# alshai/pfbwt-f

Hardware: AMD Instinct MI355X
Metric: Gbases/s end-to-end BWT+SA build; bit-exact .bwt/.sa vs reference (higher is better)
Workload: dtype u8 text / u32 indices / u64 hash; 1 GPU; S-32G; L=32000000, H=1000, seed=1000, w=10, p=100, flags=-r, uint_t=64, n=32000010000, r=83625322, input=text resident in HBM, outputs (.bwt, .ssa, .esa) left in HBM, per_rank=single GPU

## Files before the change

pfbwt-f_amd/csrc/common.h:

```cpp
#pragma once
#include <hip/hip_runtime.h>
#include <cstdint>
#include <cstdio>
#include <cstdlib>
#include <cstring>
#include <chrono>
#include <string>
#include <vector>
#include "../../include/pfbwt_hip.h"
#include "devmem.h"
#include "../../include/pfbwt_hip_dev.h"

namespace pfp {

typedef uint32_t idx_t;

constexpr int BLOCK = 256;
constexpr int WAVE = 64;

constexpr uint8_t Dollar = 2, EndOfWord = 1, EndOfDict = 0;

enum KernelId {
    K_TRIGGER_SCAN, K_PHRASE_ENDS, K_PHRASE_HASH, K_PHRASE_HASH_LONG, K_DEDUP_HEADS, K_DEDUP_LONG,
    K_DICT_BUILD, K_RADIX_HIST, K_RADIX_SCATTER, K_SCAN_REDUCE, K_SCAN_SPINE, K_SCAN_APPLY,
    K_SS_INIT_KEYS, K_SS_HEADS, K_SS_MAKE_KEYS, K_SS_WRITE_RANK, K_SS_FLAG_ACTIVE, K_COMPACT,
    K_WORD_RANK, K_PARSE_RANKS, K_DICT_SORTED, K_PBWT_ROWS, K_EMIT_COUNT, K_EMIT, K_RUNS, K_SAMPLES, K_MISC, K_EMIT_BIG, K_FILL, K_CLASS_SORT, K_FASTA, K_EMIT_LARGE, K_REC_PARSE, K_REC_DEDUP, K_REC_ASSEMBLE, K_DOC, K_LCP_PAIRS, K_LCP_LONG, K_LCP_GATHER, K_THR_TILES, K_THR_QUERIES, K_THR_LONG, K_PLCP_BUILD, K_LCP_SPARSE, K_RUN_MASKS, K_MS_INDEX, K_MS_POINTERS, K_MS_BREAKS, K_MS_LONG, K_MS_FILL, K_RI_INDEX, K_RI_SEARCH, K_RI_WALK, K_RI_ROWS,
    K_COUNT_
};
static const char *const kernel_names[K_COUNT_] = {
    "trigger_scan", "phrase_ends", "phrase_hash", "phrase_hash_long", "dedup_heads", "dedup_long",
    "dict_build", "radix_hist", "radix_scatter", "scan_reduce", "scan_spine", "scan_apply",
    "ss_init_keys", "ss_heads", "ss_make_keys", "ss_write_rank", "ss_flag_active", "compact",
    "word_rank", "parse_ranks", "dict_sorted", "pbwt_rows", "emit_count", "emit", "runs", "samples", "misc", "emit_big", "fill", "class_sort", "fasta_strip", "emit_large", "rec_parse", "rec_dedup", "rec_assemble", "doc_array", "lcp_pairs", "lcp_long", "lcp_gather", "thr_tiles", "thr_queries", "thr_long", "plcp_build", "lcp_sparse", "run_masks", "ms_index", "ms_pointers", "ms_breaks", "ms_long", "ms_fill", "ri_index", "ri_search", "ri_walk", "ri_rows"};

struct ProfRec { uint64_t launches = 0; double ms = 0, bytes = 0; };

struct Arena {
    VmRegion vm;
    char *base = nullptr;
    size_t cap = 0, lo = 0, hi = 0, want = 0;
    size_t peak_lo = 0, peak_hi_bytes = 0;
    bool failed = false;
    void reset() { lo = 0; hi = cap; failed = false; }
    void *alloc_lo(size_t bytes)
    {
        size_t a = (lo + 255) & ~(size_t)255;
        if (a + bytes > hi || !vm.commit(a, a + bytes)) { failed = true; want += bytes; return nullptr; }
        lo = a + bytes; if (lo > peak_lo) peak_lo = lo;
        return base + a;
    }
    void *alloc_hi(size_t bytes)
    {
        size_t b = (bytes + 255) & ~(size_t)255;
        if (b > hi || hi - b < lo || !vm.commit(hi - b, hi)) { failed = true; want += bytes; return nullptr; }
        hi -= b; if (cap - hi > peak_hi_bytes) peak_hi_bytes = cap - hi;
        return base + hi;
    }
    void *reserve_lo(size_t bytes)
    {
        size_t a = (lo + 255) & ~(size_t)255;
        if (a + bytes > hi) { failed = true; want += bytes; return nullptr; }
        lo = a + bytes;
        return base + a;
    }
    bool commit_range(const void *p, size_t bytes) { const size_t o = (size_t)((const char *)p - base); return vm.commit(o, o + bytes); }
    size_t offset_of(const void *p) const { return (size_t)((const char *)p - base); }
    size_t mark_hi() const { return hi; }
    void release_hi(size_t m) { hi = m; }
    size_t mark_lo() const { return lo; }
    void release_lo(size_t m) { lo = m; }
};

struct ResultSlot {
    void *p[3] = {nullptr, nullptr, nullptr};
    size_t lo_mark = (size_t)-1, lo_end = 0;
};
struct MsIndex {
    void *thr = nullptr, *lfhead = nullptr; uint8_t *head = nullptr; uint32_t *sorted = nullptr, *sym = nullptr, *dir = nullptr;
    uint32_t B = 0;
};
struct RiIndex {
    MsIndex run; void *pq = nullptr, *pv = nullptr; uint32_t *pdir = nullptr;
    uint32_t PB = 0;
};

struct Tunables {
    int verbose = 0;
    int seg_grid = 768;
    int seg_stage = 1;
    int sort_k = 0;
    int sort_no_table = 0;
    uint32_t class_sort_maxrange = 0;
    int dedup_table_log2 = 0;
    int no_trigger_table = 0;
    uint64_t emit_chunk_rows = 3ULL << 30;
    uint32_t fill_subs = 2;
    int fill_masks = 1;
    int fill_skip = 1;
    uint64_t sample_cap = ~0ULL;
    int no_runaware = 0;
    long big_group_members = -2;
    int force_wide_rows = 0;
    uint64_t ingest_block_bytes = 0;
    int expand_dma = 1;
    int ingest_readers = 0;
    uint32_t emit_group_rows = 4096;
    int dict_text_rounds = -1;
    int force_run_round = 0;
    int int_key_symbols = 3;
    int no_slot_records = 0;
    int group_reduce = 1;
    uint64_t fasta_chunk_bytes = 0;
    int parse_rec = -1;
    int parse_rec_p2 = 4;
    uint64_t parse_rec_min = 1u << 21;
    int parse_rec_depth = 1;
    uint32_t parse_rec_tile_rows = 0;
    int dict_rec = -1;
    int dict_rec_p2 = 16;
    int dedup_variant = -1;
    int64_t dedup_period = 0;
    int64_t dedup_chunk = 0;
    int dedup_packed = 1;
    int scan_waves = 16;
    int dedup_phases = 0;
    int parse_rec_table_log2 = 0;
    uint32_t doc_lds_max = 8192;
    uint32_t lcp_long_min = 512;
    uint32_t thr_long_min = 128;
    uint32_t thr_tile = 1024;
    uint64_t thr_window_rows = 1ULL << 30;
    int ms_dir_log2 = -1;
    uint32_t ms_long_min = 512;
    int ri_dir_log2 = -1;
    int ri_route = 0;
    int plcp_block_log2 = -1;
};

}

struct pfp_ctx {
    int w = 10; uint64_t p = 100; unsigned flags = 0; int device = 0;
    hipStream_t stream = nullptr;
    pfp::Arena arena;
    size_t arena_request = 0;
    uint64_t err_pos = 0; int err_ch = 0;
    pfp::VmRegion text;
    uint8_t *tb = nullptr; size_t tb_cap = 0; uint64_t n = 0; uint64_t text_hint = 0; uint64_t nseq = 0 ;
    struct RowViewPending { const uint8_t *src = nullptr; uint64_t count = 0, len = 0, stride = 0; } view;
    uint64_t left_ctx = 0;
    uint64_t tb_n = 0;
    int stage = 0;
    uint64_t m = 0, dwords = 0, dsize = 0;
    uint64_t *d_ye = nullptr;
    uint32_t *d_pid = nullptr;
    uint32_t *d_parse = nullptr;
    uint8_t *d_last = nullptr;
    uint8_t *d_dict = nullptr;
    uint32_t *d_ws = nullptr;
    uint32_t *d_wordid = nullptr;
    uint32_t *d_wrank = nullptr;
    uint32_t *d_occ = nullptr;
    uint8_t *d_sdict = nullptr;
    uint32_t *d_gsa = nullptr;
    uint8_t *d_sflag = nullptr;
    uint32_t *d_srank = nullptr;
    uint2 *d_grank = nullptr;
    bool gsa_valid = false;
    uint64_t nrows = 0;
    uint8_t *d_bwlast = nullptr; uint32_t *d_ilist = nullptr; uint64_t *d_bwsai = nullptr;
    uint8_t *d_bwl_il = nullptr;
    uint64_t nout = 0, runs = 0, esa_pairs = 0, easy = 0, hard = 0, slice_begin = 0, slice_rows = 0;
    uint8_t *d_bwt = nullptr; void *d_sa = nullptr; void *d_ssa = nullptr; void *d_esa = nullptr;
    bool have_sa = false, have_rssa = false;
    pfp::ResultSlot ma; uint64_t ma_words = 0;
    pfp::ResultSlot da;
    pfp::ResultSlot lcp;
    pfp::ResultSlot thr;
    pfp::ResultSlot msi; pfp::MsIndex msx;
    pfp::ResultSlot ms; uint64_t ms_patterns = 0, ms_bases = 0;
    std::vector<uint64_t> ms_off;
    pfp::ResultSlot rii; pfp::RiIndex rix;
    pfp::ResultSlot ri; uint64_t ri_patterns = 0, ri_reported = 0; int ri_route = 0;
    std::vector<uint64_t> ri_off;
    size_t lo_after_parse = 0, lo_after_pbwt = 0, emit_scratch_mark = 0;
    bool prof_on = false; uint64_t prof_mask = ~0ULL;
    pfp::ProfRec prof[pfp::K_COUNT_];
    struct PendingEv { hipEvent_t a, b; int id; double bytes; };
    std::vector<PendingEv> pending;
    std::vector<hipEvent_t> ev_pool;
    double stage_ms[3] = {0, 0, 0};
    int hip_err = 0;
    uint8_t *hstage[2] = {nullptr, nullptr}; hipEvent_t hstage_ev[2] = {nullptr, nullptr}; bool hstage_used[2] = {false, false};
    pfp::Tunables tun;
    struct FastaIngest {
        uint8_t *raw[2] = {nullptr, nullptr}; size_t rawcap = 0; bool used[2] = {false, false};
        hipStream_t copy = nullptr; bool copy_ready = false; hipEvent_t ev_copied[2] = {nullptr, nullptr}, ev_free[2] = {nullptr, nullptr};
        uint8_t *tiles = nullptr; size_t tiles_cap = 0;
        unsigned long long *d_tot = nullptr, *h_tot = nullptr;
        uint32_t state = 2; bool started = false; uint64_t records = 0;
        std::vector<uint64_t> rec_raw, rec_pos;
    } fa;
    uint8_t *h_bwt = nullptr; void *h_sa = nullptr;
    uint8_t *ing_buf[16] = {};
    uint64_t ing_next_off = 0;
    std::vector<std::string> doc_names; std::vector<uint64_t> doc_starts;
    uint64_t hash_seed = 0x9E3779B97F4A7C15ULL;
    int num_cus = 0;
    uint32_t *d_trigtab = nullptr;
};

namespace pfp {

inline hipEvent_t ev_get(pfp_ctx *c)
{
    if (!c->ev_pool.empty()) { hipEvent_t e = c->ev_pool.back(); c->ev_pool.pop_back(); return e; }
    hipEvent_t e; (void)hipEventCreate(&e); return e;
}
inline void prof_collect(pfp_ctx *c)
{
    if (c->pending.empty()) return;
    (void)hipStreamSynchronize(c->stream);
    for (auto &pe : c->pending) {
        float ms = 0; (void)hipEventElapsedTime(&ms, pe.a, pe.b);
        c->prof[pe.id].launches++; c->prof[pe.id].ms += ms; c->prof[pe.id].bytes += pe.bytes;
        c->ev_pool.push_back(pe.a); c->ev_pool.push_back(pe.b);
    }
    c->pending.clear();
}
struct ProfScope {
    pfp_ctx *c; int id; double bytes; hipEvent_t a = nullptr; bool on = false;
    ProfScope(pfp_ctx *c_, int id_, double bytes_) : c(c_), id(id_), bytes(bytes_)
    {
        on = c->prof_on && ((c->prof_mask >> id) & 1ULL);
        if (on) { a = ev_get(c); (void)hipEventRecord(a, c->stream); }
    }
    ~ProfScope()
    {
        if (on) {
            hipEvent_t b = ev_get(c); (void)hipEventRecord(b, c->stream);
            c->pending.push_back({a, b, id, bytes});
            if (c->pending.size() > 4096) prof_collect(c);
        }
    }
};

#define PFP_LAUNCH(ctx, id, bytes, kernel, grid, ...)                                             \
    do {                                                                                          \
        pfp::ProfScope ps_((ctx), (id), (double)(bytes));                                         \
        if ((ctx)->tun.verbose >= 3) { fprintf(stderr, "[pfbwt_hip] launch %s grid %u\n", #kernel, (unsigned)(grid)); fflush(stderr); } \
        hipLaunchKernelGGL(kernel, dim3((unsigned)(grid)), dim3(pfp::BLOCK), 0, (ctx)->stream, __VA_ARGS__); \
        hipError_t le_ = hipGetLastError();             \
        if ((ctx)->tun.verbose >= 3 && le_ == hipSuccess) le_ = hipStreamSynchronize((ctx)->stream);    \
        if (le_ != hipSuccess) { (ctx)->hip_err = (int)le_; (ctx)->err_ch = (int)le_;                 \
            fprintf(stderr, "[pfbwt_hip] launch of %s failed: %s (%s:%d)\n", #kernel, hipGetErrorString(le_), __FILE__, __LINE__); \
            return PFP_E_HIP; }                                                                       \
    } while (0)

#define PFP_LAUNCH_B(ctx, id, bytes, kernel, grid, block, ...)                                    \
    do {                                                                                          \
        pfp::ProfScope ps_((ctx), (id), (double)(bytes));                                         \
        hipLaunchKernelGGL(kernel, dim3((unsigned)(grid)), dim3((unsigned)(block)), 0, (ctx)->stream, __VA_ARGS__); \
        hipError_t le_ = hipGetLastError();                                                       \
        if (le_ != hipSuccess) { (ctx)->hip_err = (int)le_; (ctx)->err_ch = (int)le_;                 \
            fprintf(stderr, "[pfbwt_hip] launch of %s failed: %s (%s:%d)\n", #kernel, hipGetErrorString(le_), __FILE__, __LINE__); \
            return PFP_E_HIP; }                                                                       \
    } while (0)

#define PFP_HIP(ctx, expr)                                                                        \
    do {                                                                                          \
        hipError_t e_ = (expr);                                                                   \
        if (e_ != hipSuccess) { (ctx)->hip_err = (int)e_; (ctx)->err_ch = (int)e_;                \
            fprintf(stderr, "[pfbwt_hip] %s failed: %s (%s:%d)\n", #expr, hipGetErrorString(e_), __FILE__, __LINE__); \
            return PFP_E_HIP; }                                                                   \
    } while (0)

#define PFP_TRY(expr) do { int rc_ = (expr); if (rc_ != PFP_OK) return rc_; } while (0)

#define PFP_ALLOC_HI(ctx, ptr, T, count)                                                          \
    do { (ptr) = (T *)(ctx)->arena.alloc_hi(sizeof(T) * (size_t)((count) ? (count) : 1));         \
         if (!(ptr)) return PFP_E_NOMEM; } while (0)
#define PFP_ALLOC_LO(ctx, ptr, T, count)                                                          \
    do { (ptr) = (T *)(ctx)->arena.alloc_lo(sizeof(T) * (size_t)((count) ? (count) : 1));         \
         if (!(ptr)) return PFP_E_NOMEM; } while (0)

inline unsigned nblocks(uint64_t items, uint64_t per_block) { return (unsigned)((items + per_block - 1) / per_block); }
inline int bits_for(uint64_t maxval) { int b = 1; while (b < 64 && (maxval >> b)) ++b; return b; }

struct PostResult {
    pfp_ctx *c; ResultSlot &s; size_t mark;
    PostResult(pfp_ctx *c_, ResultSlot &s_) : c(c_), s(s_)
    {
        if (s.lo_mark != (size_t)-1 && c->arena.lo == s.lo_end) c->arena.release_lo(s.lo_mark);
        s = ResultSlot();
        mark = c->arena.mark_lo();
    }
    void commit(void *p0, void *p1 = nullptr, void *p2 = nullptr) { s.p[0] = p0; s.p[1] = p1; s.p[2] = p2; s.lo_mark = mark; s.lo_end = c->arena.mark_lo(); }
};
inline void drop_post_results(pfp_ctx *c) { c->ma = c->da = c->lcp = c->thr = c->msi = c->ms = ResultSlot(); c->ma_words = 0; c->msx = MsIndex(); c->ms_patterns = c->ms_bases = 0; c->ms_off.clear();
    c->rii = c->ri = ResultSlot(); c->rix = RiIndex(); c->ri_patterns = c->ri_reported = 0; c->ri_route = 0; c->ri_off.clear(); }

struct HostTimer {
    std::chrono::steady_clock::time_point t0 = std::chrono::steady_clock::now();
    double ms() const { return std::chrono::duration<double, std::milli>(std::chrono::steady_clock::now() - t0).count(); }
};

}
```

pfbwt-f_amd/csrc/dictrec.h:

```cpp
#pragma once
#include "recsort.h"

namespace pfp {

constexpr int DR_W = 4;
constexpr uint32_t DR_MAX_PHRASE = 1024;

__device__ __forceinline__ uint32_t dr_trigger(const uint8_t *D, uint64_t x, uint32_t p2)
{
    const uint8_t c = D[x];
    if (c == EndOfWord) return 1u;
    if (c == EndOfDict || x < (uint64_t)(DR_W - 1)) return 0u;
    uint32_t v = 0;
#pragma unroll
    for (int k = 0; k < DR_W; ++k) { const uint32_t b = D[x - (DR_W - 1) + k]; if (b <= 1u) return 0u; v = (v << 8) | b; }
    uint32_t h = v * 0x9E3779B1u; h ^= h >> 15; h *= 0x85EBCA77u; h ^= h >> 13;
    return (h % p2 == 0u) ? 1u : 0u;
}
__global__ __launch_bounds__(BLOCK) void k_dr_trig_count(const uint8_t *D, uint64_t N, uint32_t p2, uint32_t *cnt)
{
    __shared__ uint32_t red[4];
    const uint64_t x0 = ((uint64_t)blockIdx.x * BLOCK + threadIdx.x) * 16;
    uint32_t n = 0;
    for (int k = 0; k < 16; ++k) if (x0 + k < N) n += dr_trigger(D, x0 + k, p2);
// ... 46 lines not shown
        if (e == 0ULL) {
            e = atomicCAS(&table[slot], 0ULL, mine);
            if (e == 0ULL) { rep = 1; break; }
        }
        if ((uint32_t)(e >> 32) == tag) {
            const uint32_t r = (uint32_t)e - 1u, ra = ps[r];
            if (pe[r] - ra == b - a) {
                bool eq = true;
                for (uint32_t d = 0; d <= b - a; ++d) if (D[ra + d] != D[a + d]) { eq = false; break; }
                if (eq) break;
            }
        }
        slot = (slot + 1u) & tmask;
    }
    if (probe == REC_MAX_PROBES) atomicExch(overflow, 1u);
    eid[j] = slot; isrep[j] = rep;
}
__global__ __launch_bounds__(BLOCK) void k_dr_rep_keys(const uint8_t *D, const uint32_t *ps, const uint32_t *pe, const uint32_t *replist, uint64_t nw2, uint64_t *keys, uint32_t *vals)
{
    const uint64_t t = (uint64_t)blockIdx.x * BLOCK + threadIdx.x;
    if (t >= nw2) return;
    const uint32_t j = replist[t];
    keys[t] = dr_phrase_hash(D, ps[j], pe[j]); vals[t] = (uint32_t)t;
}
__global__ __launch_bounds__(BLOCK) void k_dr_assign_ids(const uint8_t *D, const uint32_t *sorted_t, const uint32_t *replist, const uint32_t *eid, const uint32_t *ps, const uint32_t *pe, uint64_t nw2,
                                                         uint32_t *slot2id, uint32_t *wrep, uint32_t *wlen1, uint8_t *lastw)
{
    const uint64_t i = (uint64_t)blockIdx.x * BLOCK + threadIdx.x;
    if (i > nw2) return;
    if (i == nw2) { wlen1[i] = 0u; return; }
    const uint32_t j = replist[sorted_t[i]];
    const uint32_t last = D[pe[j]] == EndOfWord ? 1u : 0u;
    slot2id[eid[j]] = (uint32_t)i; wrep[i] = j; lastw[i] = (uint8_t)last;
    wlen1[i] = pe[j] - ps[j] + 1u - last + 1u;
}
__global__ __launch_bounds__(BLOCK) void k_dr_dict_build(const uint8_t *D, const uint32_t *ps, const uint32_t *wrep, const uint32_t *wstart, uint64_t nw2, uint64_t ND, uint8_t *D2, uint32_t *wd2)
{
    const uint64_t i = (uint64_t)blockIdx.x * BLOCK + threadIdx.x;
    if (i > nw2) return;
    if (i == nw2) { D2[ND - 1] = EndOfDict; wd2[ND - 1] = (uint32_t)(nw2 ? nw2 - 1 : 0); return; }
    const uint32_t j = wrep[i], a = ps[j], o = wstart[i], L = wstart[i + 1] - o - 1u;
    for (uint32_t d = 0; d < L; ++d) { D2[o + d] = D[a + d]; wd2[o + d] = (uint32_t)i; }
    D2[o + L] = EndOfWord; wd2[o + L] = (uint32_t)i;
}
__global__ __launch_bounds__(BLOCK) void k_dr_names(const uint8_t *D, const uint32_t *pe, const uint32_t *wordid, const uint32_t *wid2, const uint32_t *wrank2, uint64_t k, uint64_t nwords, uint32_t *P2)
{
    const uint64_t j = (uint64_t)blockIdx.x * BLOCK + threadIdx.x;
    if (j < k) {
        const uint32_t e = pe[j], wj = wordid[e];
        P2[j + wj] = wrank2[wid2[j]] + 2u;
        if (D[e] == EndOfWord) P2[j + wj + 1] = 1u;
    } else if (j == k) P2[k + nwords] = 0u;
}
constexpr uint32_t DR_TIE_CAP = 1024;
__global__ __launch_bounds__(BLOCK) void k_dr_p2_heads(const uint32_t *P2, const uint32_t *SA2, uint64_t n2, uint32_t *headslot, uint8_t *open, uint32_t *nopen)
{
    __shared__ uint32_t red[4];
    const uint64_t s = (uint64_t)blockIdx.x * BLOCK + threadIdx.x;
    uint32_t op = 0u;
    if (s < n2) {
        uint32_t hd = 1u;
        if (s > 0) {
            const uint32_t x = SA2[s], y = SA2[s - 1];
            uint32_t d = 0;
            for (; d < DR_TIE_CAP; ++d) {
                const uint32_t a = x + d < n2 ? P2[x + d] : 0u, b = y + d < n2 ? P2[y + d] : 0u;
                if (a != b) { hd = (a | b) > 1u ? 1u : 0u; break; }
                if (a <= 1u) { hd = 0u; break; }
            }
            if (d == DR_TIE_CAP) { hd = 0u; op = 1u; }
        }
        headslot[s] = hd ? (uint32_t)s : 0u;
        open[s] = (uint8_t)op;
    }
    uint32_t tot;
    (void)block_excl_sum(op, red, &tot);
    if (threadIdx.x == 0 && tot) atomicAdd(nopen, tot);
}
__global__ __launch_bounds__(BLOCK) void k_dr_p2_ends(const uint32_t *P2, uint64_t n2, uint32_t *E)
{
    const uint64_t i = (uint64_t)blockIdx.x * BLOCK + threadIdx.x;
    if (i < n2) E[n2 - 1 - i] = P2[i] <= 1u ? (uint32_t)(n2 - 1 - i) : 0u;
}
__global__ __launch_bounds__(BLOCK) void k_dr_p2_double(const uint32_t *SA2, const uint32_t *rc, const uint32_t *E, uint64_t n2, uint64_t h, uint8_t *open, uint32_t *headslot, uint32_t *nopen)
{
    __shared__ uint32_t red[4];
    const uint64_t s = (uint64_t)blockIdx.x * BLOCK + threadIdx.x;
    uint32_t op = 0u;
    if (s < n2 && open[s]) {
        const uint32_t x = SA2[s], y = SA2[s - 1];
        if (rc[x + h] != rc[y + h]) headslot[s] = (uint32_t)s;
        else if (n2 - 1 - E[n2 - 1 - x] - x >= 2 * h) op = 1u;
        open[s] = (uint8_t)op;
    }
    uint32_t tot;
    (void)block_excl_sum(op, red, &tot);
    if (threadIdx.x == 0 && tot) atomicAdd(nopen, tot);
}
__global__ __launch_bounds__(BLOCK) void k_dr_p2_class(const uint32_t *SA2, const uint32_t *headslot , uint64_t n2, uint32_t *rc)
{
    const uint64_t s = (uint64_t)blockIdx.x * BLOCK + threadIdx.x;
    if (s < n2) rc[SA2[s]] = headslot[s];
}
__global__ __launch_bounds__(BLOCK) void k_dr_list_payload(const uint8_t *D, const uint32_t *inv, const uint32_t *ps, const uint32_t *pe, const uint32_t *wordid, const uint32_t *rc, uint64_t k, uint32_t *ikey, uint32_t *ipos)
{
    const uint64_t e = (uint64_t)blockIdx.x * BLOCK + threadIdx.x;
    if (e >= k) return;
    const uint32_t j = inv[e], en = pe[j];
    ikey[e] = D[en] == EndOfWord ? 0u : rc[j + 1u + wordid[en]];
    const uint32_t x = ps[j];
    ipos[e] = x | ((D[x] > EndOfWord && (x == 0 || D[x - 1] == EndOfWord)) ? 0x80000000u : 0u);
}
__global__ __launch_bounds__(BLOCK) void k_dr_slots(const uint32_t *SA2d, const uint32_t *wd2, const uint32_t *wstart, const uint8_t *lastw, const uint32_t *woff, uint64_t ND, uint32_t *rows, uint32_t *whole, uint32_t *valid)
{
    const uint64_t s = (uint64_t)blockIdx.x * BLOCK + threadIdx.x;
    if (s >= ND) return;
    const uint32_t y = SA2d[s];
    uint32_t v = 0u, r = 0u, wh = 0u;
    if (y + 1 < ND) {
        const uint32_t W = wd2[y], o = y - wstart[W], L = wstart[W + 1] - wstart[W] - 1u;
        v = lastw[W] ? 1u : (o + (uint32_t)DR_W + 1u <= L ? 1u : 0u);
        r = v ? woff[W + 1] - woff[W] : 0u;
        wh = (o == 0u && L > 0u) ? 1u : 0u;
    }
    rows[s] = r; whole[s] = wh; valid[s] = v;
}
__global__ __launch_bounds__(BLOCK) void k_dr_word_ranks(const uint32_t *SA2d, const uint32_t *wd2, const uint32_t *whole, const uint32_t *wpos, uint64_t ND, uint32_t *wrank2)
{
    const uint64_t s = (uint64_t)blockIdx.x * BLOCK + threadIdx.x;
    if (s < ND && whole[s]) wrank2[wd2[SA2d[s]]] = wpos[s];
}
__global__ __launch_bounds__(BLOCK) void k_dr_heads(const uint32_t *vlist, const uint32_t *srank2, uint64_t nv, uint32_t *head)
{
    const uint64_t v = (uint64_t)blockIdx.x * BLOCK + threadIdx.x;
    if (v >= nv) return;
    head[v] = (v == 0 || srank2[vlist[v]] != srank2[vlist[v - 1]]) ? 1u : 0u;
}
__global__ __launch_bounds__(BLOCK) void k_dr_slot_records(const uint32_t *SA2d, const uint32_t *vlist, const uint32_t *rowoff, const uint32_t *head, const uint32_t *hpos, const uint32_t *wd2, const uint32_t *wstart,
                                                           const uint32_t *woff, uint64_t nv, uint4 *srec)
{
    const uint64_t v = (uint64_t)blockIdx.x * BLOCK + threadIdx.x;
    if (v >= nv) return;
    const uint32_t s = vlist[v], y = SA2d[s], W = wd2[y];
    srec[v] = make_uint4(rowoff[s], woff[W], y - wstart[W], hpos[v] + head[v] - 1u);
}
__global__ __launch_bounds__(BLOCK) void k_dr_mark_class_rows(const uint32_t *crow, uint64_t nc, uint32_t *cstart)
{
    const uint64_t ci = (uint64_t)blockIdx.x * BLOCK + threadIdx.x;
    if (ci < nc) cstart[1u + crow[ci]] = 1u;
}
__global__ __launch_bounds__(BLOCK) void k_dr_final_heads(const uint32_t *okey, const uint32_t *cstart, uint64_t N, uint32_t *headslot)
{
    const uint64_t r = (uint64_t)blockIdx.x * BLOCK + threadIdx.x;
    if (r >= N) return;
    const bool hd = r <= 1 || cstart[r] || okey[r] != okey[r - 1];
    headslot[r] = hd ? (uint32_t)r : 0u;
}
inline int dict_sort_pfp(pfp_ctx *c, uint32_t *gsa, uint32_t *srank, uint8_t *sflag, int *taken)
{
    *taken = 0;
    const uint64_t N = c->dsize, nwords = c->dwords;
    const uint8_t *D = c->d_dict;
    const bool forced = c->tun.dict_rec > 0, verbose = c->tun.verbose != 0;
    const uint32_t p2 = c->tun.dict_rec_p2 >= 2 ? (uint32_t)c->tun.dict_rec_p2 : 16u;
    if (N < 64 || N + 64 >= 0x7FFFFFFFULL || !c->d_wordid) return PFP_OK;
    const size_t mk = c->arena.mark_hi();
    HostTimer tm;
    const unsigned gt = nblocks(N, 16 * BLOCK);
    uint32_t *bcnt, *d_cnt;
    PFP_ALLOC_HI(c, bcnt, uint32_t, gt); PFP_ALLOC_HI(c, d_cnt, uint32_t, 16);
    PFP_HIP(c, hipMemsetAsync(d_cnt, 0, 64, c->stream));
    PFP_LAUNCH(c, K_REC_PARSE, N, k_dr_trig_count, gt, D, N, p2, bcnt);
    PFP_TRY((device_scan<uint32_t, 0>(c, bcnt, bcnt, (uint64_t)gt, d_cnt)));
    uint32_t k32 = 0; PFP_TRY(d2h_u32(c, d_cnt, &k32));
    const uint64_t k = k32;
    if (k < nwords || (!forced && k * 6 > N)) { c->arena.release_hi(mk); return PFP_OK; }
    uint32_t *pe, *ps;
    PFP_ALLOC_HI(c, pe, uint32_t, k + 1); PFP_ALLOC_HI(c, ps, uint32_t, k + 1);
    PFP_LAUNCH(c, K_REC_PARSE, N + k * 4, k_dr_trig_write, gt, D, N, p2, (const uint32_t *)bcnt, pe);
    PFP_LAUNCH(c, K_REC_PARSE, k * 9, k_dr_starts, nblocks(k, BLOCK), D, (const uint32_t *)pe, k, ps, d_cnt + 1);
    uint32_t maxlen = 0; PFP_TRY(d2h_u32(c, d_cnt + 1, &maxlen));
    if (maxlen > DR_MAX_PHRASE) {
        if (verbose) fprintf(stderr, "[pfbwt_hip] recursive dictionary sort given up: a level-2 phrase of %u bytes\n", maxlen);
        c->arena.release_hi(mk); return PFP_OK;
    }
    int tl = c->tun.parse_rec_table_log2 > 0 ? c->tun.parse_rec_table_log2 : bits_for(k / 2 + 1023);
    if (tl > 31) tl = 31;
    const uint64_t tsize = 1ULL << tl;
    unsigned long long *table; uint32_t *eid, *isrep, *pos;
    PFP_ALLOC_HI(c, table, unsigned long long, tsize); PFP_ALLOC_HI(c, eid, uint32_t, k); PFP_ALLOC_HI(c, isrep, uint32_t, k); PFP_ALLOC_HI(c, pos, uint32_t, k);
    PFP_HIP(c, hipMemsetAsync(table, 0, tsize * 8, c->stream));
    PFP_LAUNCH(c, K_REC_DEDUP, N * 2 + k * 24, k_dr_dedup, nblocks(k, BLOCK), D, (const uint32_t *)ps, (const uint32_t *)pe, k, table, (uint32_t)(tsize - 1), eid, isrep, d_cnt + 3);
    uint32_t ovf = 0; PFP_TRY(d2h_u32(c, d_cnt + 3, &ovf));
    if (ovf) { if (verbose) fprintf(stderr, "[pfbwt_hip] recursive dictionary sort given up: phrase table too full\n"); c->arena.release_hi(mk); return PFP_OK; }
    uint32_t *replist; PFP_ALLOC_HI(c, replist, uint32_t, k < tsize ? k : tsize);
    PFP_TRY(device_compact(c, nullptr, isrep, k, replist, pos, d_cnt + 4));
    uint32_t nw32 = 0; PFP_TRY(d2h_u32(c, d_cnt + 4, &nw32));
    const uint64_t nw2 = nw32;
    uint32_t *slot2id, *wrep, *wstart, *wid2 = isrep, *inv0, *wid1, *inv1, *woff; uint8_t *lastw;
    PFP_ALLOC_HI(c, slot2id, uint32_t, tsize); PFP_ALLOC_HI(c, wrep, uint32_t, nw2); PFP_ALLOC_HI(c, wstart, uint32_t, nw2 + 1); PFP_ALLOC_HI(c, lastw, uint8_t, nw2 + 1);
    PFP_ALLOC_HI(c, inv0, uint32_t, k); PFP_ALLOC_HI(c, wid1, uint32_t, k); PFP_ALLOC_HI(c, inv1, uint32_t, k); PFP_ALLOC_HI(c, woff, uint32_t, nw2 + 1);
    {
        const size_t mk2 = c->arena.mark_hi();
        uint64_t *hk0, *hk1; uint32_t *hv0, *hv1;
        PFP_ALLOC_HI(c, hk0, uint64_t, nw2); PFP_ALLOC_HI(c, hk1, uint64_t, nw2); PFP_ALLOC_HI(c, hv0, uint32_t, nw2); PFP_ALLOC_HI(c, hv1, uint32_t, nw2);
        PFP_LAUNCH(c, K_REC_DEDUP, nw2 * 40, k_dr_rep_keys, nblocks(nw2, BLOCK), D, (const uint32_t *)ps, (const uint32_t *)pe, (const uint32_t *)replist, nw2, hk0, hv0);
        BitRange hr = {0, 64};
        uint64_t *sk; uint32_t *sv;
        PFP_TRY(radix_sort_pairs<uint64_t>(c, hk0, hv0, hk1, hv1, nw2, &hr, 1, &sk, &sv));
        PFP_LAUNCH(c, K_REC_DEDUP, nw2 * 24, k_dr_assign_ids, nblocks(nw2 + 1, BLOCK), D, (const uint32_t *)sv, (const uint32_t *)replist, (const uint32_t *)eid, (const uint32_t *)ps, (const uint32_t *)pe, nw2, slot2id, wrep, wstart, lastw);
        c->arena.release_hi(mk2);
    }
    PFP_TRY((device_scan<uint32_t, 0>(c, wstart, wstart, nw2 + 1, d_cnt + 5)));
    uint32_t nd32 = 0; PFP_TRY(d2h_u32(c, d_cnt + 5, &nd32));
    const uint64_t ND = (uint64_t)nd32 + 1;
    const uint64_t n2 = k + nwords + 1;
    if (verbose) fprintf(stderr, "[pfbwt_hip] recursive dictionary sort: %llu bytes, %llu words -> %llu level-2 phrases (longest %u), %llu distinct, D2 = %llu bytes (%.1f ms so far)\n",
                         (unsigned long long)N, (unsigned long long)nwords, (unsigned long long)k, maxlen, (unsigned long long)nw2, (unsigned long long)ND, tm.ms());
    if (!forced && (ND * 2 > N)) { c->arena.release_hi(mk); return PFP_OK; }
    PFP_LAUNCH(c, K_REC_DEDUP, k * 16, k_rs_wid, nblocks(k, BLOCK), (const uint32_t *)eid, (const uint32_t *)slot2id, k, wid2, eid, inv0);
    uint32_t *swid, *inv;
    {
        BitRange wr = {0, bits_for(nw2 ? nw2 - 1 : 0)};
        PFP_TRY(radix_sort_pairs<uint32_t>(c, wid2, inv0, wid1, inv1, k, &wr, 1, &swid, &inv));
        PFP_LAUNCH(c, K_REC_PARSE, k * 4, k_rs_list_bounds, nblocks(k, BLOCK), (const uint32_t *)swid, k, nw2, woff);
    }
    const uint32_t *widp = eid;
    uint8_t *D2; uint32_t *wd2, *gsa2, *srank2;
    PFP_ALLOC_HI(c, D2, uint8_t, ND + 64); PFP_ALLOC_HI(c, wd2, uint32_t, ND); PFP_ALLOC_HI(c, gsa2, uint32_t, ND); PFP_ALLOC_HI(c, srank2, uint32_t, ND);
    PFP_HIP(c, hipMemsetAsync(D2 + ND, 0, 64, c->stream));
    PFP_LAUNCH(c, K_REC_PARSE, ND * 6, k_dr_dict_build, nblocks(nw2 + 1, BLOCK), D, (const uint32_t *)ps, (const uint32_t *)wrep, (const uint32_t *)wstart, nw2, ND, D2, wd2);
    {
        const size_t mk2 = c->arena.mark_hi();
        uint64_t *k0, *k1; uint32_t *v0, *v1; uint2 *rj2;
        PFP_ALLOC_HI(c, k0, uint64_t, ND); PFP_ALLOC_HI(c, k1, uint64_t, ND); PFP_ALLOC_HI(c, v0, uint32_t, ND); PFP_ALLOC_HI(c, v1, uint32_t, ND); PFP_ALLOC_HI(c, rj2, uint2, ND);
        PFP_LAUNCH(c, K_SS_INIT_KEYS, ND * 13, k_dict_init_keys, nblocks(ND, DK_TILE), (const uint8_t *)D2, ND, k0, v0);
        BitRange full = {0, DK_KEY_BITS};
        int rounds = 0;
        PFP_TRY(suffix_sort_doubling<true>(c, ND, k0, v0, k1, v1, &full, 1, DK_CHARS, D2, gsa2, (uint32_t *)nullptr, rj2, &rounds, 9, srank2));
        c->arena.release_hi(mk2);
    }
    if (verbose) fprintf(stderr, "[pfbwt_hip]   D2 sorted (%.1f ms so far)\n", tm.ms());
    uint32_t *rows, *whole, *rowoff, *wposs, *wrank2, *P2, *SA2, *R2, *valid, *rc;
    PFP_ALLOC_HI(c, valid, uint32_t, ND); PFP_ALLOC_HI(c, rows, uint32_t, ND); PFP_ALLOC_HI(c, whole, uint32_t, ND); PFP_ALLOC_HI(c, rowoff, uint32_t, ND); PFP_ALLOC_HI(c, wposs, uint32_t, ND);
    PFP_ALLOC_HI(c, wrank2, uint32_t, nw2); PFP_ALLOC_HI(c, P2, uint32_t, n2); PFP_ALLOC_HI(c, SA2, uint32_t, n2); PFP_ALLOC_HI(c, R2, uint32_t, n2); PFP_ALLOC_HI(c, rc, uint32_t, n2);
    PFP_LAUNCH(c, K_REC_PARSE, ND * 28, k_dr_slots, nblocks(ND, BLOCK), (const uint32_t *)gsa2, (const uint32_t *)wd2, (const uint32_t *)wstart, (const uint8_t *)lastw, (const uint32_t *)woff, ND, rows, whole, valid);
    PFP_TRY((device_scan<uint32_t, 0>(c, whole, wposs, ND, nullptr)));
    PFP_LAUNCH(c, K_REC_PARSE, ND * 16, k_dr_word_ranks, nblocks(ND, BLOCK), (const uint32_t *)gsa2, (const uint32_t *)wd2, (const uint32_t *)whole, (const uint32_t *)wposs, ND, wrank2);
    PFP_LAUNCH(c, K_REC_PARSE, k * 16, k_dr_names, nblocks(k + 1, BLOCK), D, (const uint32_t *)pe, (const uint32_t *)c->d_wordid, widp, (const uint32_t *)wrank2, k, nwords, P2);
    {
        int r2 = 0;
        PFP_TRY(sort_int_suffixes(c, P2, n2, nw2 + 1, SA2, R2, &r2, 1, true));
    }
    uint8_t *open; PFP_ALLOC_HI(c, open, uint8_t, n2);
    PFP_HIP(c, hipMemsetAsync(d_cnt + 8, 0, 4, c->stream));
    PFP_LAUNCH(c, K_REC_PARSE, n2 * 17, k_dr_p2_heads, nblocks(n2, BLOCK), (const uint32_t *)P2, (const uint32_t *)SA2, n2, R2 , open, d_cnt + 8);
    PFP_TRY((device_scan<uint32_t, 1>(c, R2, R2, n2, nullptr)));
    PFP_LAUNCH(c, K_REC_PARSE, n2 * 12, k_dr_p2_class, nblocks(n2, BLOCK), (const uint32_t *)SA2, (const uint32_t *)R2, n2, rc);
    uint32_t nopen = 0; PFP_TRY(d2h_u32(c, d_cnt + 8, &nopen));
    if (nopen) {
        const uint32_t open0 = nopen;
        int rounds = 0;
        uint32_t *E; PFP_ALLOC_HI(c, E, uint32_t, n2);
        PFP_LAUNCH(c, K_REC_PARSE, n2 * 8, k_dr_p2_ends, nblocks(n2, BLOCK), (const uint32_t *)P2, n2, E);
        PFP_TRY((device_scan<uint32_t, 1>(c, E, E, n2, nullptr)));
        for (uint64_t h = DR_TIE_CAP; nopen; h *= 2, ++rounds) {
            PFP_HIP(c, hipMemsetAsync(d_cnt + 8, 0, 4, c->stream));
            PFP_LAUNCH(c, K_REC_PARSE, n2 + (uint64_t)nopen * 24, k_dr_p2_double, nblocks(n2, BLOCK), (const uint32_t *)SA2, (const uint32_t *)rc, (const uint32_t *)E, n2, h, open, R2, d_cnt + 8);
            PFP_TRY((device_scan<uint32_t, 1>(c, R2, R2, n2, nullptr)));
            PFP_LAUNCH(c, K_REC_PARSE, n2 * 12, k_dr_p2_class, nblocks(n2, BLOCK), (const uint32_t *)SA2, (const uint32_t *)R2, n2, rc);
            PFP_TRY(d2h_u32(c, d_cnt + 8, &nopen));
        }
        if (verbose) fprintf(stderr, "[pfbwt_hip]   P2 tie classes: %u neighbour pairs agree on %u symbols, resolved in %d doubling rounds\n", open0, DR_TIE_CAP, rounds);
    }
    if (verbose) fprintf(stderr, "[pfbwt_hip]   P2 sorted (%.1f ms so far)\n", tm.ms());
    uint32_t *ikey = SA2, *ipos = P2;
    PFP_LAUNCH(c, K_REC_PARSE, k * 24, k_dr_list_payload, nblocks(k, BLOCK), D, (const uint32_t *)inv, (const uint32_t *)ps, (const uint32_t *)pe, (const uint32_t *)c->d_wordid, (const uint32_t *)rc, k, ikey, ipos);
    PFP_TRY((device_scan<uint32_t, 0>(c, rows, rowoff, ND, d_cnt + 6)));
    uint32_t R32 = 0; PFP_TRY(d2h_u32(c, d_cnt + 6, &R32));
    if ((uint64_t)R32 != N - 1) { c->arena.release_hi(mk); return PFP_E_CORRUPT; }
    uint32_t *vlist, *head, *chead, *crow;
    PFP_ALLOC_HI(c, vlist, uint32_t, ND); PFP_ALLOC_HI(c, head, uint32_t, ND); PFP_ALLOC_HI(c, chead, uint32_t, ND + 1); PFP_ALLOC_HI(c, crow, uint32_t, ND + 1);
    PFP_TRY(device_compact(c, nullptr, valid, ND, vlist, wposs, d_cnt + 7));
    uint32_t nv32 = 0; PFP_TRY(d2h_u32(c, d_cnt + 7, &nv32));
    const uint64_t nv = nv32;
    uint4 *srec; PFP_ALLOC_HI(c, srec, uint4, nv);
    PFP_LAUNCH(c, K_REC_PARSE, nv * 12, k_dr_heads, nblocks(nv, BLOCK), (const uint32_t *)vlist, (const uint32_t *)srank2, nv, head);
    PFP_HIP(c, hipMemsetAsync(d_cnt, 0, 32, c->stream));
    PFP_TRY(device_compact(c, nullptr, head, nv, chead, wposs, d_cnt));
    PFP_LAUNCH(c, K_REC_PARSE, nv * 44, k_dr_slot_records, nblocks(nv, BLOCK), (const uint32_t *)gsa2, (const uint32_t *)vlist, (const uint32_t *)rowoff, (const uint32_t *)head, (const uint32_t *)wposs, (const uint32_t *)wd2,
               (const uint32_t *)wstart, (const uint32_t *)woff, nv, srec);
    uint32_t nc32 = 0; PFP_TRY(d2h_u32(c, d_cnt, &nc32));
    const uint64_t nc = nc32;
    PFP_LAUNCH(c, K_REC_PARSE, nc * 24, k_rs_class_rows, nblocks(nc + 1, BLOCK), (const uint32_t *)chead, (const uint4 *)srec, nc, nv, N - 1, crow, chead + nc);
    uint32_t tile_rows = c->tun.parse_rec_tile_rows ? c->tun.parse_rec_tile_rows : (uint32_t)RS_TILE;
    if (tile_rows > (uint32_t)RS_TILE) tile_rows = RS_TILE;
    if (tile_rows < 2) tile_rows = 2;
    const int keybits = bits_for(n2);
    uint32_t *bigc, *okey, *cstart;
    PFP_ALLOC_HI(c, bigc, uint32_t, nc + 1); PFP_ALLOC_HI(c, okey, uint32_t, N); PFP_ALLOC_HI(c, cstart, uint32_t, N + 1);
    PFP_HIP(c, hipMemsetAsync(cstart, 0, (N + 1) * 4, c->stream));
    const unsigned ga = nblocks(N - 1, RS_TILE / 2);
    PFP_LAUNCH(c, K_REC_ASSEMBLE, (N - 1) * 16 + nv * 16, (k_rs_assemble<false, true>), ga, (const uint4 *)srec, (const uint32_t *)chead, (const uint32_t *)crow, (uint32_t)nc, (const uint32_t *)ikey, (const uint32_t *)ipos,
               keybits, tile_rows, gsa, (uint32_t *)nullptr, bigc, d_cnt + 1, okey, sflag);
    PFP_LAUNCH(c, K_MISC, 8, k_rs_first_row, 1, gsa, (uint32_t *)nullptr, N);
    uint32_t nb32 = 0; PFP_TRY(d2h_u32(c, d_cnt + 1, &nb32));
    if (nb32) {
        const uint64_t nb = nb32;
        uint32_t *bigoff; PFP_ALLOC_HI(c, bigoff, uint32_t, nb + 1);
        PFP_LAUNCH(c, K_REC_PARSE, nb * 12, k_rs_big_sizes, nblocks(nb + 1, BLOCK), (const uint32_t *)bigc, nb, (const uint32_t *)crow, bigoff);
        PFP_TRY((device_scan<uint32_t, 0>(c, bigoff, bigoff, nb + 1, d_cnt + 2)));
        uint32_t nbr32 = 0; PFP_TRY(d2h_u32(c, d_cnt + 2, &nbr32));
        const uint64_t nbr = nbr32;
        if (verbose) fprintf(stderr, "[pfbwt_hip]   assembly: %llu classes with more than %u rows (%llu rows) through the global sort\n", (unsigned long long)nb, tile_rows, (unsigned long long)nbr);
        uint64_t *bk0, *bk1; uint32_t *bv0, *bv1;
        PFP_ALLOC_HI(c, bk0, uint64_t, nbr); PFP_ALLOC_HI(c, bk1, uint64_t, nbr); PFP_ALLOC_HI(c, bv0, uint32_t, nbr); PFP_ALLOC_HI(c, bv1, uint32_t, nbr);
        PFP_LAUNCH(c, K_REC_PARSE, nbr * 40, k_rs_big_rows, nblocks(nbr, BLOCK), (const uint32_t *)bigc, (const uint32_t *)bigoff, (uint32_t)nb, nbr, (const uint32_t *)crow, (const uint32_t *)chead, (const uint4 *)srec,
                   (const uint32_t *)ikey, (const uint32_t *)ipos, bk0, bv0, 1);
        BitRange br[2] = {{0, keybits}, {32, 32 + bits_for(nb - 1)}};
        uint64_t *sk; uint32_t *sv;
        PFP_TRY(radix_sort_pairs<uint64_t>(c, bk0, bv0, bk1, bv1, nbr, br, 2, &sk, &sv));
        PFP_LAUNCH(c, K_REC_PARSE, nbr * 24, (k_rs_big_store<false, true>), nblocks(nbr, BLOCK), (const uint64_t *)sk, (const uint32_t *)sv, nbr, (const uint32_t *)bigc, (const uint32_t *)bigoff, (const uint32_t *)crow, gsa,
                   (uint32_t *)nullptr, okey, sflag);
    }
    PFP_LAUNCH(c, K_REC_PARSE, nc * 8, k_dr_mark_class_rows, nblocks(nc, BLOCK), (const uint32_t *)crow, nc, cstart);
    PFP_LAUNCH(c, K_REC_PARSE, N * 12, k_dr_final_heads, nblocks(N, BLOCK), (const uint32_t *)okey, (const uint32_t *)cstart, N, srank);
    PFP_TRY((device_scan<uint32_t, 1>(c, srank, srank, N, nullptr)));
    PFP_HIP(c, hipMemsetAsync(sflag, 0, 1, c->stream));
    PFP_HIP(c, hipStreamSynchronize(c->stream));
    if (verbose) fprintf(stderr, "[pfbwt_hip]   dictionary assembled: %llu slots, %llu D2 classes (%.1f ms)\n", (unsigned long long)nv, (unsigned long long)nc, tm.ms());
    c->arena.release_hi(mk);
    *taken = 1;
    return PFP_OK;
}

}
```

pfbwt-f_amd/csrc/pfbwt_hip.hip:

```cpp
#include "common.h"
#include "prims.h"
#include "parse.h"
#include "fasta.h"
#include "sufsort.h"
#include "recsort.h"
#include "dictrec.h"
#include "emit.h"
#include "markers.h"
#include "docarray.h"
#include "lcparray.h"
#include "thresholds.h"
#include "matchstats.h"
#include "runindex.h"
#include <algorithm>
#include <functional>
#include <map>
#include <sched.h>
#include <thread>
#if defined(__SSE2__)
#include <emmintrin.h>
#endif

using namespace pfp;

#ifndef PFP_BACKEND_NAME
#define PFP_BACKEND_NAME "hip-gfx950"
#endif

static int ensure_arena(pfp_ctx *c, uint64_t n_hint)
{
    size_t want = c->arena_request ? c->arena_request : (size_t)(96ULL * n_hint + (64ULL << 20));
    if (!c->arena_request) {
        size_t fr = 0, tot = 0;
        if (hipMemGetInfo(&fr, &tot) == hipSuccess) {
            const size_t avail = fr + c->arena.vm.committed;
            const size_t cap = avail - avail / 16;
            if (want > cap) want = cap;
        }
    }
    want &= ~(size_t)4095;
    if (c->arena.base && c->arena.cap >= want) return PFP_OK;
    VmRegion nv;
    if (nv.reserve(want, c->device) != hipSuccess) { c->arena.want = want; return PFP_E_NOMEM; }
    if (c->arena.base) { PFP_HIP(c, hipStreamSynchronize(c->stream)); (void)hipDeviceSynchronize(); c->arena.vm.destroy(); c->arena.base = nullptr; c->arena.cap = 0; }
    c->arena.vm = nv; nv.base = nullptr;
    c->arena.base = c->arena.vm.base; c->arena.cap = want; c->arena.reset();
    return PFP_OK;
}

static int ensure_text(pfp_ctx *c, uint64_t need_n)
{
    const size_t need = 16 + (((size_t)need_n + 4095) / 4096) * 4096 + 4096 + 64;
    if (c->tb && c->tb_cap >= need) return PFP_OK;
    if (!c->text.live() || need > c->text.va_bytes) {
        size_t fr = 0, tot = 0;
        if (hipMemGetInfo(&fr, &tot) != hipSuccess) { (void)hipGetLastError(); tot = (size_t)1 << 38; }
        size_t va = c->text_hint ? (size_t)c->text_hint + (size_t)c->text_hint / 8 + ((size_t)64 << 20) : (4 * need > ((size_t)64 << 20) ? 4 * need : ((size_t)64 << 20));
        if (!c->text_hint && c->text.live() && va < 2 * c->text.va_bytes) va = 2 * c->text.va_bytes;
        if (!c->text_hint && va > tot && tot > need + need / 4) va = tot;
        if (va < need) va = need + need / 4;
        VmRegion nr;
        if (nr.reserve(va, c->device) != hipSuccess) return PFP_E_NOMEM;
        if (c->tb) {
            if (!nr.commit(0, 16 + (size_t)c->n)) { nr.destroy(); return PFP_E_NOMEM; }
            PFP_HIP(c, hipMemcpyAsync(nr.base, c->tb, 16 + (size_t)c->n, hipMemcpyDeviceToDevice, c->stream));
            PFP_HIP(c, hipStreamSynchronize(c->stream));
            c->text.destroy();
        }
        c->text = nr; nr.base = nullptr;
        c->tb = (uint8_t *)c->text.base; c->tb_cap = 0;
    }
    if (!c->text.commit(0, need)) return PFP_E_NOMEM;
    c->tb_cap = c->text.vmm ? (c->text.lo_edge < c->text.va_bytes ? c->text.lo_edge : c->text.va_bytes) : c->text.va_bytes;
    return PFP_OK;
}

static void reset_results(pfp_ctx *c)
{
    c->stage = 0; c->n = 0; c->nseq = 0; c->tb_n = 0; c->left_ctx = 0; c->view.src = nullptr; c->m = c->dwords = c->dsize = 0; c->nrows = 0; c->nout = c->runs = c->esa_pairs = 0;
    c->gsa_valid = false; c->d_wrank = nullptr; c->d_bwt = nullptr; c->d_sa = c->d_ssa = c->d_esa = nullptr;
    c->d_bwlast = nullptr; c->d_ilist = nullptr; c->d_bwsai = nullptr; c->d_bwl_il = nullptr;
    drop_post_results(c);
    c->d_ye = nullptr; c->d_pid = nullptr; c->d_parse = nullptr; c->d_last = nullptr; c->d_dict = nullptr; c->d_ws = nullptr; c->d_wordid = nullptr;
    c->d_occ = nullptr; c->d_sdict = nullptr; c->d_gsa = nullptr; c->d_grank = nullptr; c->d_srank = nullptr; c->d_sflag = nullptr;
    c->arena.reset();
    c->fa.started = false; c->fa.state = 2; c->fa.records = 0; c->fa.rec_raw.clear(); c->fa.rec_pos.clear();
}

static const char *const tunable_names[] = {"verbose", "seg_grid", "seg_stage", "sort_k", "sort_no_table", "class_sort_maxrange", "dedup_table_log2", "no_trigger_table",
                                            "emit_chunk_rows", "fill_subs", "sample_cap", "no_runaware", "big_group_members", "force_wide_rows", "fasta_chunk_bytes", "ingest_block_bytes", "emit_group_rows", "no_slot_records", "dict_text_rounds", "int_key_symbols", "force_run_round",
                                            "ingest_readers", "expand_dma", "parse_rec", "parse_rec_p2", "parse_rec_min", "parse_rec_depth", "parse_rec_tile_rows", "parse_rec_table_log2", "dict_rec", "dict_rec_p2", "dedup_variant", "dedup_phases", "dedup_period", "dedup_chunk", "doc_lds_max", "dedup_packed", "group_reduce", "scan_waves", "lcp_long_min", "thr_long_min", "thr_tile", "thr_window_rows", "plcp_block_log2", "fill_masks", "fill_skip", "ms_dir_log2", "ms_long_min", "ri_dir_log2", "ri_route"};
static int set_tunable(pfp_ctx *c, const char *key, long long v)
{
    Tunables &t = c->tun;
    if (!strcmp(key, "verbose")) t.verbose = (int)v;
    else if (!strcmp(key, "seg_grid")) t.seg_grid = (int)v;
    else if (!strcmp(key, "seg_stage")) t.seg_stage = (int)v;
    else if (!strcmp(key, "sort_k")) t.sort_k = (int)v;
    else if (!strcmp(key, "sort_no_table")) t.sort_no_table = (int)v;
    else if (!strcmp(key, "class_sort_maxrange")) t.class_sort_maxrange = (uint32_t)v;
    else if (!strcmp(key, "dedup_table_log2")) t.dedup_table_log2 = (int)v;
    else if (!strcmp(key, "no_trigger_table")) t.no_trigger_table = (int)v;
    else if (!strcmp(key, "emit_chunk_rows")) t.emit_chunk_rows = v > 0 ? (uint64_t)v : (3ULL << 30);
    else if (!strcmp(key, "fill_subs")) t.fill_subs = (uint32_t)v;
    else if (!strcmp(key, "fill_masks")) t.fill_masks = (int)v;
    else if (!strcmp(key, "fill_skip")) t.fill_skip = (int)v;
    else if (!strcmp(key, "sample_cap")) t.sample_cap = v < 0 ? ~0ULL : (uint64_t)v;
    else if (!strcmp(key, "no_runaware")) t.no_runaware = (int)v;
    else if (!strcmp(key, "big_group_members")) t.big_group_members = (long)v;
    else if (!strcmp(key, "force_wide_rows")) t.force_wide_rows = (int)v;
    else if (!strcmp(key, "fasta_chunk_bytes")) t.fasta_chunk_bytes = v > 0 ? (uint64_t)v : 0;
    else if (!strcmp(key, "ingest_block_bytes")) t.ingest_block_bytes = v > 0 ? (uint64_t)v : 0;
    else if (!strcmp(key, "emit_group_rows")) t.emit_group_rows = v > 0 ? (uint32_t)v : 0u;
    else if (!strcmp(key, "no_slot_records")) t.no_slot_records = (int)v;
    else if (!strcmp(key, "dict_text_rounds")) t.dict_text_rounds = (int)v;
    else if (!strcmp(key, "int_key_symbols")) t.int_key_symbols = (int)v;
    else if (!strcmp(key, "force_run_round")) t.force_run_round = (int)v;
    else if (!strcmp(key, "ingest_readers")) t.ingest_readers = (int)v;
    else if (!strcmp(key, "expand_dma")) t.expand_dma = (int)v;
    else if (!strcmp(key, "parse_rec")) t.parse_rec = (int)v;
    else if (!strcmp(key, "parse_rec_p2")) t.parse_rec_p2 = (int)v;
    else if (!strcmp(key, "parse_rec_min")) t.parse_rec_min = v > 0 ? (uint64_t)v : 0;
    else if (!strcmp(key, "parse_rec_depth")) t.parse_rec_depth = (int)v;
    else if (!strcmp(key, "parse_rec_tile_rows")) t.parse_rec_tile_rows = v > 0 ? (uint32_t)v : 0u;
    else if (!strcmp(key, "parse_rec_table_log2")) t.parse_rec_table_log2 = (int)v;
    else if (!strcmp(key, "dict_rec")) t.dict_rec = (int)v;
    else if (!strcmp(key, "dict_rec_p2")) t.dict_rec_p2 = (int)v;
    else if (!strcmp(key, "dedup_variant")) t.dedup_variant = (int)v;
    else if (!strcmp(key, "dedup_phases")) t.dedup_phases = (int)v;
    else if (!strcmp(key, "dedup_packed")) t.dedup_packed = (int)v;
    else if (!strcmp(key, "group_reduce")) t.group_reduce = (int)v;
    else if (!strcmp(key, "scan_waves")) t.scan_waves = (int)v;
    else if (!strcmp(key, "dedup_period")) t.dedup_period = (int64_t)v;
    else if (!strcmp(key, "dedup_chunk")) t.dedup_chunk = (int64_t)v;
    else if (!strcmp(key, "doc_lds_max")) t.doc_lds_max = v < 2 ? 2u : v > (long long)DOC_LDS_CAP ? DOC_LDS_CAP : (uint32_t)v;
    else if (!strcmp(key, "lcp_long_min")) t.lcp_long_min = v < 16 ? 16u : v > (1LL << 30) ? (1u << 30) : (((uint32_t)v + 15u) & ~15u);
    else if (!strcmp(key, "thr_long_min")) t.thr_long_min = v < 1 ? 1u : v > (1LL << 30) ? (1u << 30) : (uint32_t)v;
    else if (!strcmp(key, "thr_tile")) { uint32_t p2 = 16; while (p2 < (1u << 20) && (long long)p2 < v) p2 *= 2; t.thr_tile = p2; }
    else if (!strcmp(key, "thr_window_rows")) t.thr_window_rows = v < 1 ? (1ULL << 30) : (uint64_t)v;
    else if (!strcmp(key, "plcp_block_log2")) t.plcp_block_log2 = v < 0 ? -1 : v > PLCP_BLOCK_LOG2_MAX ? PLCP_BLOCK_LOG2_MAX : (int)v;
    else if (!strcmp(key, "ms_dir_log2")) t.ms_dir_log2 = v < 0 ? -1 : v > MS_DIR_LOG2_MAX ? MS_DIR_LOG2_MAX : (int)v;
    else if (!strcmp(key, "ms_long_min")) t.ms_long_min = v < 1 ? 1u : v > (1LL << 30) ? (1u << 30) : (uint32_t)v;
    else if (!strcmp(key, "ri_dir_log2")) t.ri_dir_log2 = v < 0 ? -1 : v > RI_DIR_LOG2_MAX ? RI_DIR_LOG2_MAX : (int)v;
    else if (!strcmp(key, "ri_route")) t.ri_route = v < 0 ? 0 : v > 2 ? 2 : (int)v;
    else return PFP_E_ARG;
    return PFP_OK;
}
static void load_tunables_from_env(pfp_ctx *c)
{
    if (getenv("PFP_VERBOSE")) c->tun.verbose = 1;
    const char *hooks = getenv("PFP_TEST_HOOKS");
    if (!hooks || strcmp(hooks, "1")) return;
    for (const char *name : tunable_names) {
        char env[64] = "PFP_"; size_t k = 4;
        for (const char *q = name; *q && k + 1 < sizeof env; ++q) env[k++] = (char)((*q >= 'a' && *q <= 'z') ? *q - 32 : *q);
        env[k] = 0;
        const char *e = getenv(env);
        if (e) (void)set_tunable(c, name, *e ? atoll(e) : 1LL);
    }
}

extern "C" {

const char *pfp_backend(void) { return PFP_BACKEND_NAME; }
int pfp_debug_set(pfp_ctx *c, const char *key, long long value) { return (c && key) ? set_tunable(c, key, value) : PFP_E_ARG; }

const char *pfp_strerror(int s)
{
    switch (s) {
    case PFP_OK: return "ok";
    case PFP_E_ARG: return "invalid argument";
    case PFP_E_INVALID_CHAR: return "error, invalid character";
    case PFP_E_TOO_LARGE: return "input too long for 32-bit device indices";
    case PFP_E_NOMEM: return "device workspace exhausted";
    case PFP_E_HIP: return "HIP runtime error";
    case PFP_E_ONE_WORD: return "error: only one dict word total. Re-run with a smaller p modulus";
    case PFP_E_STATE: return "call order violated";
    case PFP_E_CORRUPT: return "something went wrong!";
    case PFP_E_IO: return "failed to open file!";
    default: return "unknown status";
    }
}

pfp_ctx *pfp_create(int w, uint64_t p, unsigned flags, int device, uint64_t workspace_bytes, int *status)
{
    int st = PFP_OK;
    pfp_ctx *c = nullptr;
    if (w < 1 || w > 32 || p == 0) st = PFP_E_ARG;
    else {
        int ndev = 0;
        if (hipGetDeviceCount(&ndev) != hipSuccess || ndev <= 0 || device < 0 || device >= ndev) st = PFP_E_HIP;
        else if (hipSetDevice(device) != hipSuccess) st = PFP_E_HIP;
        else {
            c = new pfp_ctx();
            c->w = w; c->p = p; c->flags = flags; c->device = device; c->arena_request = (size_t)workspace_bytes;
            load_tunables_from_env(c);
            if (hipStreamCreateWithFlags(&c->stream, hipStreamNonBlocking) != hipSuccess) { delete c; c = nullptr; st = PFP_E_HIP; }
        }
    }
    if (status) *status = st;
    return c;
}

void pfp_destroy(pfp_ctx *c)
{
    if (!c) return;
    (void)hipSetDevice(c->device);
    if (c->stream) (void)hipStreamSynchronize(c->stream);
    (void)hipDeviceSynchronize();
    prof_collect(c);
    for (auto e : c->ev_pool) (void)hipEventDestroy(e);
    c->text.destroy();
    for (int k = 0; k < 2; ++k) { if (c->fa.raw[k]) (void)hipFree(c->fa.raw[k]); if (c->fa.ev_copied[k]) (void)hipEventDestroy(c->fa.ev_copied[k]); if (c->fa.ev_free[k]) (void)hipEventDestroy(c->fa.ev_free[k]); }
    if (c->fa.tiles) (void)hipFree(c->fa.tiles);
    if (c->fa.d_tot) (void)hipFree(c->fa.d_tot);
    if (c->fa.h_tot) (void)hipHostFree(c->fa.h_tot);
    if (c->fa.copy_ready) (void)hipStreamDestroy(c->fa.copy);
    for (auto &q : c->ing_buf) if (q) (void)hipHostFree(q);
    if (c->d_trigtab) (void)hipFree(c->d_trigtab);
    for (int k = 0; k < 2; ++k) { if (c->hstage[k]) (void)hipHostFree(c->hstage[k]); if (c->hstage_ev[k]) (void)hipEventDestroy(c->hstage_ev[k]); }
    c->arena.vm.destroy();
    if (c->stream) (void)hipStreamDestroy(c->stream);
    delete c;
}

int pfp_error_detail(pfp_ctx *c, uint64_t *pos, int *ch)
{
    if (!c) return PFP_E_ARG;
    if (pos) *pos = c->err_pos;
    if (ch) *ch = c->err_ch;
    return PFP_OK;
}
uint64_t pfp_workspace_needed(pfp_ctx *c) { return c ? (uint64_t)(c->arena.cap + c->arena.want) : 0; }
int pfp_reset(pfp_ctx *c)
{
    if (!c) return PFP_E_ARG;
    PFP_HIP(c, hipSetDevice(c->device));
    PFP_HIP(c, hipStreamSynchronize(c->stream));
    reset_results(c);
    return PFP_OK;
}

int pfp_profile_enable(pfp_ctx *c, int on) { if (!c) return PFP_E_ARG; prof_collect(c); c->prof_on = on != 0; c->prof_mask = ~0ULL; return PFP_OK; }
int pfp_profile_select(pfp_ctx *c, const char *kernel)
{
    if (!c || !kernel) return PFP_E_ARG;
    prof_collect(c);
    for (int i = 0; i < K_COUNT_; ++i) if (!strcmp(kernel, kernel_names[i])) { c->prof_on = true; c->prof_mask = 1ULL << i; return PFP_OK; }
    return PFP_E_ARG;
}
int pfp_profile_reset(pfp_ctx *c) { if (!c) return PFP_E_ARG; prof_collect(c); for (auto &r : c->prof) r = ProfRec(); return PFP_OK; }
int pfp_profile_get(pfp_ctx *c, int idx, const char **name, uint64_t *launches, double *ms, double *bytes)
{
    if (!c || idx < 0 || idx >= K_COUNT_) return PFP_E_ARG;
    prof_collect(c);
    if (name) *name = kernel_names[idx];
    if (launches) *launches = c->prof[idx].launches;
    if (ms) *ms = c->prof[idx].ms;
    if (bytes) *bytes = c->prof[idx].bytes;
    return PFP_OK;
}
int pfp_stage_ms(pfp_ctx *c, double out[3]) { if (!c || !out) return PFP_E_ARG; for (int i = 0; i < 3; ++i) out[i] = c->stage_ms[i]; return PFP_OK; }

constexpr size_t STAGE_BYTES = (size_t)32 << 20;
static bool host_pointer_is_pinned(const void *p)
{
    hipPointerAttribute_t a;
    if (hipPointerGetAttributes(&a, p) == hipSuccess) return a.type == hipMemoryTypeHost;
    (void)hipGetLastError();
    return false;
}
static int h2d_copy(pfp_ctx *c, uint8_t *dst, const uint8_t *src, uint64_t len, bool *in_flight = nullptr)
{
    if (in_flight) *in_flight = false;
    if (!len) return PFP_OK;
    if (host_pointer_is_pinned(src)) { PFP_HIP(c, hipMemcpyAsync(dst, src, (size_t)len, hipMemcpyHostToDevice, c->stream)); if (in_flight) *in_flight = true; else PFP_HIP(c, hipStreamSynchronize(c->stream)); return PFP_OK; }
    if (len <= ((size_t)1 << 16)) { PFP_HIP(c, hipMemcpyAsync(dst, src, (size_t)len, hipMemcpyHostToDevice, c->stream)); PFP_HIP(c, hipStreamSynchronize(c->stream)); return PFP_OK; }
    for (int k = 0; k < 2; ++k) if (!c->hstage[k]) {
        PFP_HIP(c, hipHostMalloc((void **)&c->hstage[k], STAGE_BYTES, hipHostMallocDefault));
        PFP_HIP(c, hipEventCreate(&c->hstage_ev[k]));
    }
    int k = 0;
    for (uint64_t off = 0; off < len; off += STAGE_BYTES, k ^= 1) {
        const size_t chunk = (size_t)(len - off < STAGE_BYTES ? len - off : STAGE_BYTES);
        if (c->hstage_used[k]) PFP_HIP(c, hipEventSynchronize(c->hstage_ev[k]));
        memcpy(c->hstage[k], src + off, chunk);
        PFP_HIP(c, hipMemcpyAsync(dst + off, c->hstage[k], chunk, hipMemcpyHostToDevice, c->stream));
        PFP_HIP(c, hipEventRecord(c->hstage_ev[k], c->stream));
        c->hstage_used[k] = true;
    }
    return PFP_OK;
}
static int feed_common(pfp_ctx *c, const void *src, uint64_t len, int end_of_seq, hipMemcpyKind kind)
{
    if (!c || (!src && len)) return PFP_E_ARG;
    PFP_HIP(c, hipSetDevice(c->device));
    if (c->stage != 0) reset_results(c);
    const uint64_t add = len + (end_of_seq ? (uint64_t)c->w : 0);
    if (c->n + add + (uint64_t)c->w + 64 >= ((c->flags & PFP_FLAG_U64) ? (1ULL << 40) : 0xFFFFFFFFULL)) return PFP_E_TOO_LARGE;
    PFP_TRY(ensure_text(c, c->n + add + (uint64_t)c->w));
    bool in_flight = false;
    if (len && kind == hipMemcpyHostToDevice) PFP_TRY(h2d_copy(c, c->tb + 16 + c->n, (const uint8_t *)src, len, &in_flight));
    else if (len) PFP_HIP(c, hipMemcpyAsync(c->tb + 16 + c->n, src, (size_t)len, kind, c->stream));
    c->n += len;
    if (end_of_seq) {
        ++c->nseq;
        PFP_HIP(c, hipMemsetAsync(c->tb + 16 + c->n, 'A', (size_t)c->w, c->stream));
        c->n += (uint64_t)c->w;
    }
    if (in_flight || (len && kind == hipMemcpyDeviceToDevice)) PFP_HIP(c, hipStreamSynchronize(c->stream));
    c->tb_n = c->n;
    return PFP_OK;
}
int pfp_parse_reopen(pfp_ctx *c)
{
    if (!c) return PFP_E_ARG;
    PFP_HIP(c, hipSetDevice(c->device));
    if (c->stage == 0) return PFP_OK;
    if (!c->tb || !c->tb_n || c->tb_n != c->n) return PFP_E_STATE;
    PFP_HIP(c, hipStreamSynchronize(c->stream));
    const uint64_t n = c->n, nseq = c->nseq;
    reset_results(c);
    c->nseq = nseq;
    c->n = c->tb_n = n;
    return PFP_OK;
}
static int flush_view(pfp_ctx *c);
int pfp_text_view(pfp_ctx *c, const uint8_t **d_text, uint64_t *n)
{
    if (!c || !d_text || !n) return PFP_E_ARG;
    PFP_TRY(flush_view(c));
    if (!c->tb || c->tb_n != c->n) { *d_text = nullptr; *n = 0; return PFP_OK; }
    PFP_HIP(c, hipSetDevice(c->device));
    PFP_HIP(c, hipStreamSynchronize(c->stream));
    *d_text = c->tb + 16; *n = c->n;
    return PFP_OK;
}
int pfp_parse_feed_left_context(pfp_ctx *c)
{
    if (!c) return PFP_E_ARG;
    if (c->stage != 0) { PFP_HIP(c, hipSetDevice(c->device)); reset_results(c); }
    if (c->n != 0) return PFP_E_STATE;
    const std::vector<uint8_t> a((size_t)c->w, (uint8_t)'A');
    PFP_TRY(feed_common(c, a.data(), a.size(), 0, hipMemcpyHostToDevice));
    c->left_ctx = (uint64_t)c->w;
    return PFP_OK;
}
static int flush_view(pfp_ctx *c)
{
    if (!c->view.src) return PFP_OK;
    const uint64_t count = c->view.count, len = c->view.len;
    const uint64_t blocks_per_row = ((len + 15) / 16 + BLOCK - 1) / BLOCK;
    PFP_LAUNCH(c, K_MISC, 2 * count * len, k_feed_batch, count * blocks_per_row, c->view.src, count, len, c->view.stride, c->w, c->tb + 16);
    c->view.src = nullptr;
    return PFP_OK;
}
int pfp_parse_feed_device_view(pfp_ctx *c, const void *d_bases, uint64_t count, uint64_t len, uint64_t stride)
{
    if (!c || !d_bases || !count || !len || stride < len) return PFP_E_ARG;
    PFP_HIP(c, hipSetDevice(c->device));
    if (c->stage != 0) reset_results(c);
    if (c->n != 0) return PFP_E_STATE;
    const uint64_t pitch = len + (uint64_t)c->w, add = count * pitch;
    if (add + (uint64_t)c->w + 64 >= ((c->flags & PFP_FLAG_U64) ? (1ULL << 40) : 0xFFFFFFFFULL)) return PFP_E_TOO_LARGE;
    const uint64_t blocks_per_row = ((len + 15) / 16 + BLOCK - 1) / BLOCK;
    if (count * blocks_per_row >= 0x7FFFFFFFULL) return PFP_E_TOO_LARGE;
    PFP_TRY(ensure_text(c, add + (uint64_t)c->w));
    c->view.src = (const uint8_t *)d_bases; c->view.count = count; c->view.len = len; c->view.stride = stride;
    c->n = add; c->tb_n = c->n; c->nseq = count;
    return PFP_OK;
}
int pfp_parse_feed(pfp_ctx *c, const uint8_t *bases, uint64_t len, int end_of_seq) { if (c) PFP_TRY(flush_view(c)); return feed_common(c, bases, len, end_of_seq, hipMemcpyHostToDevice); }
int pfp_parse_feed_device(pfp_ctx *c, const void *d_bases, uint64_t len, int end_of_seq) { if (c) PFP_TRY(flush_view(c)); return feed_common(c, d_bases, len, end_of_seq, hipMemcpyDeviceToDevice); }
int pfp_parse_feed_device_batch(pfp_ctx *c, const void *d_bases, uint64_t count, uint64_t len, uint64_t stride)
{
    if (!c || (!d_bases && count && len) || stride < len) return PFP_E_ARG;
    if (!count) return PFP_OK;
    PFP_TRY(flush_view(c));
    if (!len) { for (uint64_t k = 0; k < count; ++k) PFP_TRY(feed_common(c, nullptr, 0, 1, hipMemcpyDeviceToDevice)); return PFP_OK; }
    PFP_HIP(c, hipSetDevice(c->device));
    if (c->stage != 0) reset_results(c);
    const uint64_t pitch = len + (uint64_t)c->w, add = count * pitch;
    if (c->n + add + (uint64_t)c->w + 64 >= ((c->flags & PFP_FLAG_U64) ? (1ULL << 40) : 0xFFFFFFFFULL)) return PFP_E_TOO_LARGE;
    PFP_TRY(ensure_text(c, c->n + add + (uint64_t)c->w));
    uint8_t *dst = c->tb + 16 + c->n;
    const uint64_t blocks_per_row = ((len + 15) / 16 + BLOCK - 1) / BLOCK;
    if (count * blocks_per_row >= 0x7FFFFFFFULL) return PFP_E_TOO_LARGE;
    PFP_LAUNCH(c, K_MISC, 2 * count * len, k_feed_batch, count * blocks_per_row, (const uint8_t *)d_bases, count, len, stride, c->w, dst);
    c->n += add; c->tb_n = c->n; c->nseq += count;
    return PFP_OK;
}

int pfp_parse_feed_batch(pfp_ctx *c, const uint8_t *bases, uint64_t count, uint64_t len, uint64_t stride)
{
    if (!c || (!bases && count && len) || stride < len) return PFP_E_ARG;
    if (!count) return PFP_OK;
    PFP_TRY(flush_view(c));
    if (!len || !host_pointer_is_pinned(bases)) {
        for (uint64_t k = 0; k < count; ++k) PFP_TRY(feed_common(c, bases + k * stride, len, 1, hipMemcpyHostToDevice));
        return PFP_OK;
    }
    PFP_HIP(c, hipSetDevice(c->device));
    if (c->stage != 0) reset_results(c);
    const uint64_t pitch = len + (uint64_t)c->w, add = count * pitch;
    if (c->n + add + (uint64_t)c->w + 64 >= ((c->flags & PFP_FLAG_U64) ? (1ULL << 40) : 0xFFFFFFFFULL)) return PFP_E_TOO_LARGE;
    PFP_TRY(ensure_text(c, c->n + add + (uint64_t)c->w));
    uint8_t *dst = c->tb + 16 + c->n;
    for (uint64_t k = 0; k < count; ++k) PFP_HIP(c, hipMemcpyAsync(dst + k * pitch, bases + k * stride, (size_t)len, hipMemcpyHostToDevice, c->stream));
    PFP_LAUNCH(c, K_MISC, count * (uint64_t)c->w, k_pad_rows, nblocks(count * (uint64_t)c->w, BLOCK), dst, count, len, pitch, c->w);
    PFP_HIP(c, hipStreamSynchronize(c->stream));
    c->n += add; c->tb_n = c->n; c->nseq += count;
    return PFP_OK;
}

constexpr size_t FA_RAW_MAX = (size_t)256 << 20, FA_RAW_MIN = (size_t)1 << 20;
int pfp_parse_reserve(pfp_ctx *c, uint64_t text_bytes)
{
    if (!c) return PFP_E_ARG;
    if (!c->text.live()) c->text_hint = text_bytes;
    return PFP_OK;
}
static int ensure_copy_stream(pfp_ctx *c)
{
    auto &f = c->fa;
    if (f.copy_ready) return PFP_OK;
    PFP_HIP(c, hipStreamCreateWithFlags(&f.copy, hipStreamNonBlocking));
    f.copy_ready = true;
// ... 1442 lines not shown
```

pfbwt-f_amd/csrc/recsort.h:

```cpp
#pragma once
#include "sufsort.h"

namespace pfp {

constexpr uint32_t REC_MAX_PHRASE = 1024;
constexpr int RS_TRIG_PER = 16;
constexpr int RS_TRIG_TILE = BLOCK * RS_TRIG_PER;

__device__ __forceinline__ uint32_t rs_trigger(uint32_t s, uint32_t p2)
{
    uint32_t h = s * 0x9E3779B1u; h ^= h >> 15; h *= 0x85EBCA77u; h ^= h >> 13;
    return (h % p2 == 0u) ? 1u : 0u;
}
__device__ __forceinline__ uint32_t rs_trig_mask16(const uint32_t *S, uint64_t N, uint64_t i0, uint32_t p2)
{
    uint32_t m = 0;
    if (i0 + RS_TRIG_PER <= N) {
        const uint4 *q = reinterpret_cast<const uint4 *>(S + i0);
#pragma unroll
        for (int v = 0; v < 4; ++v) {
            const uint4 a = q[v];
            m |= (rs_trigger(a.x, p2) | (rs_trigger(a.y, p2) << 1) | (rs_trigger(a.z, p2) << 2) | (rs_trigger(a.w, p2) << 3)) << (4 * v);
        }
    } else {
        for (int k = 0; k < RS_TRIG_PER; ++k) if (i0 + k < N) m |= rs_trigger(S[i0 + k], p2) << k;
    }
    if (i0 == 0) m &= ~1u;
    if (N - 1 >= i0 && N - 1 < i0 + RS_TRIG_PER) m |= 1u << (uint32_t)(N - 1 - i0);
    return m;
}
__global__ __launch_bounds__(BLOCK) void k_rs_trig_count(const uint32_t *S, uint64_t N, uint32_t p2, uint32_t *cnt)
{
    __shared__ uint32_t red[4];
    const uint64_t i0 = ((uint64_t)blockIdx.x * BLOCK + threadIdx.x) * RS_TRIG_PER;
    const uint32_t m = i0 < N ? rs_trig_mask16(S, N, i0, p2) : 0u;
    uint32_t tot;
    (void)block_excl_sum((uint32_t)__popc(m), red, &tot);
    if (threadIdx.x == 0) cnt[blockIdx.x] = tot;
}
__global__ __launch_bounds__(BLOCK) void k_rs_trig_write(const uint32_t *S, uint64_t N, uint32_t p2, const uint32_t *blockoff, uint32_t *ps)
{
    __shared__ uint32_t red[4];
    const uint64_t i0 = ((uint64_t)blockIdx.x * BLOCK + threadIdx.x) * RS_TRIG_PER;
    uint32_t m = i0 < N ? rs_trig_mask16(S, N, i0, p2) : 0u;
    uint32_t tot;
    uint32_t o = 1u + blockoff[blockIdx.x] + block_excl_sum((uint32_t)__popc(m), red, &tot);
    while (m) { const int b = __ffs((int)m) - 1; ps[o++] = (uint32_t)(i0 + (uint32_t)b); m &= m - 1u; }
    if (blockIdx.x == 0 && threadIdx.x == 0) ps[0] = 0u;
}
__global__ __launch_bounds__(BLOCK) void k_rs_max_phrase(const uint32_t *ps, uint64_t k, uint32_t *out)
{
    __shared__ uint32_t red[4];
    const uint64_t j = (uint64_t)blockIdx.x * BLOCK + threadIdx.x;
    const uint32_t len = j < k ? ps[j + 1] - ps[j] + 1u : 0u;
    uint32_t tot;
    (void)block_incl_max(len, red, &tot);
    if (threadIdx.x == 0 && tot > *(volatile uint32_t *)out) atomicMax(out, tot);
}

constexpr uint32_t REC_MAX_PROBES = 128;
__device__ __forceinline__ uint64_t rs_phrase_hash(const uint32_t *S, uint32_t a, uint32_t b)
{
    uint64_t h = 0x243F6A8885A308D3ULL;
    for (uint32_t i = a; i <= b; ++i) { h = (h ^ S[i]) * 0x9E3779B97F4A7C15ULL; h ^= h >> 29; }
    h *= 0xBF58476D1CE4E5B9ULL; h ^= h >> 32;
    return h;
}
__global__ __launch_bounds__(BLOCK) void k_rs_dedup(const uint32_t *S, const uint32_t *ps, uint64_t k, unsigned long long *table, uint32_t tmask, uint32_t *eid, uint32_t *isrep, uint32_t *overflow)
{
    const uint64_t j = (uint64_t)blockIdx.x * BLOCK + threadIdx.x;
    if (j >= k) return;
    const uint32_t a = ps[j], b = ps[j + 1];
    const uint64_t h = rs_phrase_hash(S, a, b);
    const uint32_t tag = (uint32_t)(h >> 32);
    const unsigned long long mine = ((unsigned long long)tag << 32) | (unsigned long long)(a + 1u);
    uint32_t slot = (uint32_t)h & tmask, rep = 0, probe = 0;
    for (; probe < REC_MAX_PROBES; ++probe) {
        unsigned long long e = table[slot];
        if (e == 0ULL) {
            e = atomicCAS(&table[slot], 0ULL, mine);
            if (e == 0ULL) { rep = 1; break; }
        }
        if ((uint32_t)(e >> 32) == tag) {
            const uint32_t ra = (uint32_t)e - 1u;
            bool eq = true;
            for (uint32_t d = 0; d <= b - a; ++d) if (S[ra + d] != S[a + d]) { eq = false; break; }
            if (eq) break;
        }
        slot = (slot + 1u) & tmask;
    }
    if (probe == REC_MAX_PROBES) atomicExch(overflow, 1u);
    eid[j] = slot; isrep[j] = rep;
}
__global__ __launch_bounds__(BLOCK) void k_rs_rep_keys(const uint32_t *S, const uint32_t *ps, const uint32_t *replist, uint64_t nw, uint64_t k, uint64_t *keys, uint32_t *vals)
{
    const uint64_t t = (uint64_t)blockIdx.x * BLOCK + threadIdx.x;
    if (t >= nw) return;
    const uint32_t j = replist[t];
    keys[t] = (uint64_t)j + 1 == k ? ~0ULL : (rs_phrase_hash(S, ps[j], ps[j + 1]) >> 1);
    vals[t] = (uint32_t)t;
}
__global__ __launch_bounds__(BLOCK) void k_rs_assign_ids(const uint32_t *sorted_t, const uint32_t *replist, const uint32_t *eid, const uint32_t *ps, uint64_t nw, uint32_t *slot2id, uint32_t *wrep, uint32_t *wlen1)
{
    const uint64_t i = (uint64_t)blockIdx.x * BLOCK + threadIdx.x;
    if (i > nw) return;
    if (i == nw) { wlen1[i] = 0u; return; }
    const uint32_t j = replist[sorted_t[i]];
    slot2id[eid[j]] = (uint32_t)i; wrep[i] = j;
    wlen1[i] = ps[j + 1] - ps[j] + 2u;
}
__global__ __launch_bounds__(BLOCK) void k_rs_wid(const uint32_t *eid, const uint32_t *slot2id, uint64_t k, uint32_t *wid, uint32_t *wid_keep, uint32_t *idx)
{
    const uint64_t j = (uint64_t)blockIdx.x * BLOCK + threadIdx.x;
    if (j < k) { const uint32_t id = slot2id[eid[j]]; wid[j] = id; wid_keep[j] = id; idx[j] = (uint32_t)j; }
}
__global__ __launch_bounds__(BLOCK) void k_rs_dict_build(const uint32_t *S, const uint32_t *ps, const uint32_t *wrep, const uint32_t *wstart, uint64_t nw, uint32_t *D, uint32_t *wd)
{
    const uint64_t i = (uint64_t)blockIdx.x * BLOCK + threadIdx.x;
    if (i >= nw) return;
    const uint32_t j = wrep[i], a = ps[j], L = ps[j + 1] - a + 1u, o = wstart[i];
    for (uint32_t d = 0; d < L; ++d) { D[o + d] = S[a + d] + 2u; wd[o + d] = (uint32_t)i; }
    D[o + L] = i + 1 == nw ? 0u : 1u; wd[o + L] = (uint32_t)i;
}
__global__ __launch_bounds__(BLOCK) void k_rs_list_bounds(const uint32_t *skeys, uint64_t k, uint64_t nw, uint32_t *woff)
{
    const uint64_t e = (uint64_t)blockIdx.x * BLOCK + threadIdx.x;
    if (e >= k) return;
    const uint32_t id = skeys[e];
    if (e == 0 || skeys[e - 1] != id) woff[id] = (uint32_t)e;
    if (e + 1 == k) woff[nw] = (uint32_t)k;
}
__global__ __launch_bounds__(BLOCK) void k_rs_slots(const uint32_t *SAD, const uint32_t *wd, const uint32_t *wstart, const uint32_t *woff, uint64_t ND, uint32_t *rows, uint32_t *whole, uint32_t *valid)
{
    const uint64_t s = (uint64_t)blockIdx.x * BLOCK + threadIdx.x;
    if (s >= ND) return;
    const uint32_t x = SAD[s], i = wd[x], o = x - wstart[i], L = wstart[i + 1] - wstart[i] - 1u;
    rows[s] = o + 1u < L ? woff[i + 1] - woff[i] : 0u;
    valid[s] = o + 1u < L ? 1u : 0u;
    whole[s] = o == 0u ? 1u : 0u;
}
__global__ __launch_bounds__(BLOCK) void k_rs_word_ranks(const uint32_t *SAD, const uint32_t *wd, const uint32_t *whole, const uint32_t *wpos, uint64_t ND, uint32_t *wrank)
{
    const uint64_t s = (uint64_t)blockIdx.x * BLOCK + threadIdx.x;
    if (s < ND && whole[s]) wrank[wd[SAD[s]]] = wpos[s] + 1u;
}
__global__ __launch_bounds__(BLOCK) void k_rs_names(const uint32_t *wid, const uint32_t *wrank, uint64_t k, uint32_t *P2)
{
    const uint64_t j = (uint64_t)blockIdx.x * BLOCK + threadIdx.x;
    if (j < k) P2[j] = wrank[wid[j]];
    else if (j == k) P2[j] = 0u;
}
__global__ __launch_bounds__(BLOCK) void k_rs_list_payload(const uint32_t *inv, const uint32_t *R2, const uint32_t *ps, uint64_t k, uint32_t *ikey, uint32_t *ipos)
{
    const uint64_t e = (uint64_t)blockIdx.x * BLOCK + threadIdx.x;
    if (e >= k) return;
    const uint32_t j = inv[e];
    ikey[e] = R2[j + 1]; ipos[e] = ps[j];
}
__global__ __launch_bounds__(BLOCK) void k_rs_heads(const uint32_t *D, const uint32_t *SAD, const uint32_t *vlist, uint64_t nv, uint32_t *head)
{
    const uint64_t v = (uint64_t)blockIdx.x * BLOCK + threadIdx.x;
    if (v >= nv) return;
    const uint32_t s = vlist[v];
    const uint32_t sp = v ? vlist[v - 1] : 0u;
    uint32_t hd = (v == 0 || sp + 1u != s) ? 1u : 0u;
    uint32_t x = SAD[s], y = SAD[s ? s - 1 : 0];
    if (!hd) {
        for (uint32_t d = 0; d <= REC_MAX_PHRASE + 1u; ++d) {
            const uint32_t a = D[x + d], b = D[y + d];
            if (a != b) { hd = (a | b) > 1u ? 1u : 0u; break; }
            if (a <= 1u) break;
        }
    }
    head[v] = hd;
}
__global__ __launch_bounds__(BLOCK) void k_rs_slot_records(const uint32_t *SAD, const uint32_t *vlist, const uint32_t *rowoff, const uint32_t *head, const uint32_t *hpos , const uint32_t *wd, const uint32_t *wstart,
                                                            const uint32_t *woff, uint64_t nv, uint4 *srec)
{
    const uint64_t v = (uint64_t)blockIdx.x * BLOCK + threadIdx.x;
    if (v >= nv) return;
    const uint32_t s = vlist[v], x = SAD[s], i = wd[x];
    srec[v] = make_uint4(rowoff[s], woff[i], x - wstart[i], hpos[v] + head[v] - 1u);
}
__global__ __launch_bounds__(BLOCK) void k_rs_class_rows(const uint32_t *chead, const uint4 *srec, uint64_t nc, uint64_t nv, uint64_t R, uint32_t *crow, uint32_t *chead_end)
{
    const uint64_t ci = (uint64_t)blockIdx.x * BLOCK + threadIdx.x;
    if (ci < nc) crow[ci] = srec[chead[ci]].x;
    else if (ci == nc) { crow[ci] = (uint32_t)R; *chead_end = (uint32_t)nv; }
}

__device__ __forceinline__ uint32_t rs_lower_bound(const uint32_t *a, uint32_t lo, uint32_t hi, uint64_t key)
{
    while (lo < hi) { const uint32_t mid = lo + ((hi - lo) >> 1); if ((uint64_t)a[mid] < key) lo = mid + 1; else hi = mid; }
    return lo;
}

template <int NB> __device__ __forceinline__ void rs_same_digit_lanes(uint32_t d, uint32_t &plo, uint32_t &phi)
{
#pragma unroll
    for (int bb = 0; bb < NB; ++bb) {
        const uint32_t neg = (uint32_t)(((int32_t)(d << (31 - bb))) >> 31);
        const unsigned long long m = __builtin_amdgcn_ballot_w64(neg != 0u);
        plo &= ~((uint32_t)m ^ neg); phi &= ~((uint32_t)(m >> 32) ^ neg);
    }
}

constexpr int RA_DB = 9, RA_RADIX = 1 << RA_DB;
template <bool RANK, bool KEYOUT> __global__ __launch_bounds__(BLOCK) void k_rs_assemble(const uint4 *srec, const uint32_t *chead , const uint32_t *crow , uint32_t nc,
                                                                            const uint32_t *ikey, const uint32_t *ipos, int keybits, uint32_t tile_rows, uint32_t *SA, uint32_t *rank,
                                                                            uint32_t *bigc, uint32_t *nbig, uint32_t *okey ,
                                                                            uint8_t *oflag )
{
    constexpr int ITEMS = RS_ITEMS, TILE = RS_TILE;
    constexpr uint32_t STEP = TILE / 2;
    __shared__ uint32_t wh[BLOCK / WAVE][RA_RADIX];
    __shared__ uint64_t skeys[TILE];
    __shared__ uint16_t sidx[TILE];
    __shared__ uint16_t srow[TILE + 1];
    __shared__ uint32_t red[4];
    __shared__ uint32_t ctl[4];
    const int lane = threadIdx.x & 63, wave = threadIdx.x >> 6;
    const uint64_t w0 = (uint64_t)blockIdx.x * STEP;
    if (threadIdx.x == 0) { ctl[0] = rs_lower_bound(crow, 0u, nc, w0); ctl[1] = rs_lower_bound(crow, 0u, nc, w0 + STEP); }
    __syncthreads();
    uint32_t ci = ctl[0];
    const uint32_t ci1 = ctl[1];
    while (ci < ci1) {
        __syncthreads();
        if (threadIdx.x == 0) {
            const uint64_t lim = (uint64_t)crow[ci] + tile_rows;
            uint32_t lo = ci, hi = ci1;
            while (lo < hi) { const uint32_t mid = lo + ((hi - lo + 1) >> 1); if ((uint64_t)crow[mid] <= lim) lo = mid; else hi = mid - 1; }
            ctl[2] = lo;
            if (lo == ci) bigc[atomicAdd(nbig, 1u)] = ci;
        }
        __syncthreads();
        const uint32_t cj = ctl[2];
        if (cj == ci) { ++ci; continue; }
        const uint32_t r0 = crow[ci], n = crow[cj] - r0, v0 = chead[ci], ns = chead[cj] - v0;
        for (uint32_t t = threadIdx.x; t < ns; t += BLOCK) srow[t] = (uint16_t)(srec[v0 + t].x - r0);
        if (threadIdx.x == 0) srow[ns] = (uint16_t)n;
        __syncthreads();
        const uint32_t nit = (n + BLOCK - 1) / BLOCK;
        uint32_t xi[ITEMS];
#pragma unroll
        for (int it = 0; it < ITEMS; ++it) {
            const uint32_t i = threadIdx.x + (uint32_t)it * BLOCK;
            xi[it] = 0u;
            if (i < n) {
                uint32_t lo = 0, hi = ns - 1;
                while (lo < hi) { const uint32_t mid = lo + ((hi - lo + 1) >> 1); if (srow[mid] <= i) lo = mid; else hi = mid - 1; }
                const uint4 rec = srec[v0 + lo];
                const uint32_t e = rec.y + (i - (rec.x - r0));
                xi[it] = KEYOUT ? (rec.z ? (ipos[e] & 0x7FFFFFFFu) + rec.z : ipos[e]) : ipos[e] + rec.z;
                skeys[i] = ((uint64_t)(rec.w - ci) << keybits) | ikey[e];
                sidx[i] = (uint16_t)i;
            }
        }
        for (uint32_t i = n + threadIdx.x; i < nit * BLOCK; i += BLOCK) { skeys[i] = ~0ULL; sidx[i] = (uint16_t)i; }
        __syncthreads();
        int tbits = keybits;
        for (uint32_t hs = cj - 1 - ci; hs; hs >>= 1) ++tbits;
        const int npass = (tbits + RA_DB - 1) / RA_DB;
        const uint32_t base = (uint32_t)wave * (nit * WAVE) + lane;
        for (int p = 0; p < npass; ++p) {
            const int sh = RA_DB * p;
            uint64_t kk[ITEMS]; uint16_t vv[ITEMS]; unsigned dg[ITEMS];
#pragma unroll
            for (int w = 0; w < BLOCK / WAVE; ++w) { wh[w][threadIdx.x] = 0; wh[w][threadIdx.x + BLOCK] = 0; }
            __syncthreads();
#pragma unroll
            for (int it = 0; it < ITEMS; ++it) {
                if ((uint32_t)it < nit) {
                    const uint32_t i = base + (uint32_t)it * WAVE;
                    kk[it] = skeys[i]; vv[it] = sidx[i];
                    const uint32_t d = (uint32_t)(kk[it] >> sh) & (RA_RADIX - 1);
                    uint32_t plo = 0xFFFFFFFFu, phi = 0xFFFFFFFFu;
                    rs_same_digit_lanes<RA_DB>(d, plo, phi);
                    const int leader = plo ? __builtin_ctz(plo) : 32 + __builtin_ctz(phi);
                    uint32_t old = 0;
                    if (lane == leader) { old = wh[wave][d]; wh[wave][d] = old + (uint32_t)__builtin_popcount(plo) + (uint32_t)__builtin_popcount(phi); }
                    old = __shfl(old, leader);
                    dg[it] = d | ((old + __builtin_amdgcn_mbcnt_hi(phi, __builtin_amdgcn_mbcnt_lo(plo, 0u))) << RA_DB);
                }
            }
            __syncthreads();
            {
                const unsigned d0 = 2u * threadIdx.x;
                uint32_t c0[BLOCK / WAVE], c1[BLOCK / WAVE]; uint32_t total = 0;
#pragma unroll
                for (int w = 0; w < BLOCK / WAVE; ++w) { const uint2 q = *reinterpret_cast<const uint2 *>(&wh[w][d0]); c0[w] = q.x; c1[w] = q.y; total += q.x + q.y; }
                uint32_t tt;
                uint32_t run = block_excl_sum(total, red, &tt);
                uint32_t o0[BLOCK / WAVE];
#pragma unroll
                for (int w = 0; w < BLOCK / WAVE; ++w) { o0[w] = run; run += c0[w]; }
#pragma unroll
                for (int w = 0; w < BLOCK / WAVE; ++w) { *reinterpret_cast<uint2 *>(&wh[w][d0]) = make_uint2(o0[w], run); run += c1[w]; }
            }
            __syncthreads();
#pragma unroll
            for (int it = 0; it < ITEMS; ++it) {
                if ((uint32_t)it < nit) {
                    const uint32_t li = wh[wave][dg[it] & (RA_RADIX - 1)] + (dg[it] >> RA_DB);
                    skeys[li] = kk[it]; sidx[li] = vv[it];
                }
            }
            __syncthreads();
        }
        if (KEYOUT) {
            const uint64_t km = keybits >= 32 ? 0xFFFFFFFFULL : ((1ULL << keybits) - 1ULL);
            for (uint32_t i = threadIdx.x; i < n; i += BLOCK) okey[1u + r0 + i] = (uint32_t)(skeys[i] & km);
            __syncthreads();
        }
        uint32_t *sx = reinterpret_cast<uint32_t *>(skeys);
#pragma unroll
        for (int it = 0; it < ITEMS; ++it) { const uint32_t i = threadIdx.x + (uint32_t)it * BLOCK; if (i < n) sx[i] = xi[it]; }
        __syncthreads();
        for (uint32_t i = threadIdx.x; i < n; i += BLOCK) {
            uint32_t x = sx[sidx[i]];
            if (KEYOUT) { oflag[1u + r0 + i] = (uint8_t)(x >> 31); x &= 0x7FFFFFFFu; }
            SA[1u + r0 + i] = x;
            if (RANK) rank[x] = 1u + r0 + i;
        }
        ci = cj;
    }
}

__global__ __launch_bounds__(BLOCK) void k_rs_big_sizes(const uint32_t *bigc, uint64_t nb, const uint32_t *crow, uint32_t *sizes)
{
    const uint64_t b = (uint64_t)blockIdx.x * BLOCK + threadIdx.x;
    if (b < nb) sizes[b] = crow[bigc[b] + 1] - crow[bigc[b]];
    else if (b == nb) sizes[b] = 0u;
}
__global__ __launch_bounds__(BLOCK) void k_rs_big_rows(const uint32_t *bigc, const uint32_t *bigoff , uint32_t nb, uint64_t nbr, const uint32_t *crow, const uint32_t *chead, const uint4 *srec,
                                                       const uint32_t *ikey, const uint32_t *ipos, uint64_t *keys, uint32_t *vals, int flagged )
{
    const uint64_t q = (uint64_t)blockIdx.x * BLOCK + threadIdx.x;
    if (q >= nbr) return;
    uint32_t lo = 0, hi = nb - 1;
    while (lo < hi) { const uint32_t mid = lo + ((hi - lo + 1) >> 1); if ((uint64_t)bigoff[mid] <= q) lo = mid; else hi = mid - 1; }
    const uint32_t b = lo, c = bigc[b], row = crow[c] + (uint32_t)(q - bigoff[b]);
    uint32_t vl = chead[c], vh = chead[c + 1] - 1;
    while (vl < vh) { const uint32_t mid = vl + ((vh - vl + 1) >> 1); if (srec[mid].x <= row) vl = mid; else vh = mid - 1; }
    const uint4 rec = srec[vl];
    const uint32_t e = rec.y + (row - rec.x);
    keys[q] = ((uint64_t)b << 32) | ikey[e];
    vals[q] = flagged ? (rec.z ? (ipos[e] & 0x7FFFFFFFu) + rec.z : ipos[e]) : ipos[e] + rec.z;
}
template <bool RANK, bool KEYOUT> __global__ __launch_bounds__(BLOCK) void k_rs_big_store(const uint64_t *keys, const uint32_t *vals, uint64_t nbr, const uint32_t *bigc, const uint32_t *bigoff, const uint32_t *crow, uint32_t *SA, uint32_t *rank, uint32_t *okey, uint8_t *oflag)
{
    const uint64_t q = (uint64_t)blockIdx.x * BLOCK + threadIdx.x;
    if (q >= nbr) return;
    const uint32_t b = (uint32_t)(keys[q] >> 32);
    const uint32_t row = crow[bigc[b]] + (uint32_t)(q - bigoff[b]);
    uint32_t x = vals[q];
    if (KEYOUT) { oflag[1u + row] = (uint8_t)(x >> 31); x &= 0x7FFFFFFFu; }
    SA[1u + row] = x;
    if (RANK) rank[x] = 1u + row;
    if (KEYOUT) okey[1u + row] = (uint32_t)keys[q];
}
__global__ __launch_bounds__(BLOCK) void k_rs_first_row(uint32_t *SA, uint32_t *rank, uint64_t N)
{
    if (blockIdx.x == 0 && threadIdx.x == 0) { SA[0] = (uint32_t)(N - 1); if (rank) rank[N - 1] = 0u; }
}

inline int sort_int_suffixes(pfp_ctx *c, const uint32_t *dS, uint64_t N, uint64_t maxsym, uint32_t *SA, uint32_t *rank, int *rounds, int depth = 0, bool want_rank = true);

inline int sort_int_suffixes_doubling(pfp_ctx *c, const uint32_t *dS, uint64_t N, uint64_t maxsym, uint32_t *SA, uint32_t *rank, int *rounds)
{
    const size_t mk = c->arena.mark_hi();
    uint64_t *k0, *k1; uint32_t *v0, *v1;
    PFP_ALLOC_HI(c, k0, uint64_t, N); PFP_ALLOC_HI(c, k1, uint64_t, N);
    PFP_ALLOC_HI(c, v0, uint32_t, N); PFP_ALLOC_HI(c, v1, uint32_t, N);
    const int sb = bits_for(maxsym);
    const int nsym = (c->tun.int_key_symbols == 3 && 3 * sb <= 64) ? 3 : 2;
    PFP_LAUNCH(c, K_SS_INIT_KEYS, N * 16, k_int_init_keys, nblocks(N, BLOCK), dS, N, sb, nsym, k0, v0);
    BitRange rr = {0, nsym * sb};
    PFP_TRY(suffix_sort_doubling<false>(c, N, k0, v0, k1, v1, &rr, 1, (uint32_t)nsym, (const uint8_t *)nullptr, SA, rank, (uint2 *)nullptr, rounds));
    c->arena.release_hi(mk);
    return PFP_OK;
}

inline int suffix_sort_pfp(pfp_ctx *c, const uint32_t *dS, uint64_t N, uint64_t maxsym, uint32_t *SA, uint32_t *rank , int depth, int *taken)
{
    *taken = 0;
    const bool forced = c->tun.parse_rec > 0, verbose = c->tun.verbose != 0;
    const uint32_t p2 = c->tun.parse_rec_p2 >= 2 ? (uint32_t)c->tun.parse_rec_p2 : 4u;
    if (N < 8 || N + 64 >= 0xFFFFFFFFULL || maxsym + 2 >= 0xFFFFFFFFULL) return PFP_OK;
    const size_t mk = c->arena.mark_hi();
    HostTimer tm;
    const unsigned gt = nblocks(N, RS_TRIG_TILE);
    uint32_t *bcnt, *d_cnt;
    PFP_ALLOC_HI(c, bcnt, uint32_t, gt); PFP_ALLOC_HI(c, d_cnt, uint32_t, 8);
    PFP_HIP(c, hipMemsetAsync(d_cnt, 0, 32, c->stream));
    PFP_LAUNCH(c, K_REC_PARSE, N * 4, k_rs_trig_count, gt, dS, N, p2, bcnt);
    PFP_TRY((device_scan<uint32_t, 0>(c, bcnt, bcnt, (uint64_t)gt, d_cnt)));
    uint32_t k32 = 0; PFP_TRY(d2h_u32(c, d_cnt, &k32));
    const uint64_t k = k32;
    if (k < 2 || (!forced && k * 2 > N)) { c->arena.release_hi(mk); return PFP_OK; }
    if (N + 2 * k >= 0xFFFFFFFFULL) {
        if (verbose) fprintf(stderr, "[pfbwt_hip] recursive parse sort given up: N + 2 * %llu phrases do not fit 32 bits\n", (unsigned long long)k);
        c->arena.release_hi(mk); return PFP_OK;
    }
    uint32_t *ps; PFP_ALLOC_HI(c, ps, uint32_t, k + 1);
    PFP_LAUNCH(c, K_REC_PARSE, N * 4 + k * 4, k_rs_trig_write, gt, dS, N, p2, (const uint32_t *)bcnt, ps);
    PFP_LAUNCH(c, K_REC_PARSE, k * 4, k_rs_max_phrase, nblocks(k, BLOCK), (const uint32_t *)ps, k, d_cnt + 1);
    uint32_t maxlen = 0; PFP_TRY(d2h_u32(c, d_cnt + 1, &maxlen));
    if (maxlen > REC_MAX_PHRASE) {
        if (verbose) fprintf(stderr, "[pfbwt_hip] recursive parse sort given up: a level-2 phrase of %u symbols\n", maxlen);
        c->arena.release_hi(mk); return PFP_OK;
    }
    int tl = c->tun.parse_rec_table_log2 > 0 ? c->tun.parse_rec_table_log2 : bits_for(k / 8 + 1023);
    if (tl > 31) tl = 31;
    const uint64_t tsize = 1ULL << tl;
    unsigned long long *table; uint32_t *eid, *isrep, *pos;
    PFP_ALLOC_HI(c, table, unsigned long long, tsize); PFP_ALLOC_HI(c, eid, uint32_t, k); PFP_ALLOC_HI(c, isrep, uint32_t, k); PFP_ALLOC_HI(c, pos, uint32_t, k);
    PFP_HIP(c, hipMemsetAsync(table, 0, tsize * 8, c->stream));
    PFP_LAUNCH(c, K_REC_DEDUP, N * 8 + k * 24, k_rs_dedup, nblocks(k, BLOCK), dS, (const uint32_t *)ps, k, table, (uint32_t)(tsize - 1), eid, isrep, d_cnt + 3);
    uint32_t ovf = 0; PFP_TRY(d2h_u32(c, d_cnt + 3, &ovf));
    if (ovf) {
        if (verbose) fprintf(stderr, "[pfbwt_hip] recursive parse sort given up: the table of %llu slots is too full for the distinct level-2 phrases among %llu\n", (unsigned long long)tsize, (unsigned long long)k);
        c->arena.release_hi(mk); return PFP_OK;
    }
    uint32_t *replist; PFP_ALLOC_HI(c, replist, uint32_t, k < tsize ? k : tsize);
    PFP_TRY(device_compact(c, nullptr, isrep, k, replist, pos, d_cnt + 4));
    uint32_t nw32 = 0; PFP_TRY(d2h_u32(c, d_cnt + 4, &nw32));
    const uint64_t nw = nw32;
    uint32_t *slot2id, *wrep, *wstart, *wid = isrep , *inv0, *wid1, *inv1, *woff;
    PFP_ALLOC_HI(c, slot2id, uint32_t, tsize); PFP_ALLOC_HI(c, wrep, uint32_t, nw); PFP_ALLOC_HI(c, wstart, uint32_t, nw + 1);
    PFP_ALLOC_HI(c, inv0, uint32_t, k); PFP_ALLOC_HI(c, wid1, uint32_t, k); PFP_ALLOC_HI(c, inv1, uint32_t, k); PFP_ALLOC_HI(c, woff, uint32_t, nw + 1);
    {
        const size_t mk2 = c->arena.mark_hi();
        uint64_t *hk0, *hk1; uint32_t *hv0, *hv1;
        PFP_ALLOC_HI(c, hk0, uint64_t, nw); PFP_ALLOC_HI(c, hk1, uint64_t, nw); PFP_ALLOC_HI(c, hv0, uint32_t, nw); PFP_ALLOC_HI(c, hv1, uint32_t, nw);
        PFP_LAUNCH(c, K_REC_DEDUP, nw * 40, k_rs_rep_keys, nblocks(nw, BLOCK), dS, (const uint32_t *)ps, (const uint32_t *)replist, nw, k, hk0, hv0);
        BitRange hr = {0, 64};
        uint64_t *sk; uint32_t *sv;
        PFP_TRY(radix_sort_pairs<uint64_t>(c, hk0, hv0, hk1, hv1, nw, &hr, 1, &sk, &sv));
        PFP_LAUNCH(c, K_REC_DEDUP, nw * 24, k_rs_assign_ids, nblocks(nw + 1, BLOCK), (const uint32_t *)sv, (const uint32_t *)replist, (const uint32_t *)eid, (const uint32_t *)ps, nw, slot2id, wrep, wstart);
        c->arena.release_hi(mk2);
    }
    PFP_TRY((device_scan<uint32_t, 0>(c, wstart, wstart, nw + 1, d_cnt + 5)));
    uint32_t nd32 = 0; PFP_TRY(d2h_u32(c, d_cnt + 5, &nd32));
    const uint64_t ND = nd32;
    if (verbose) fprintf(stderr, "[pfbwt_hip] recursive parse sort (depth %d): N=%llu -> %llu phrases (longest %u), %llu distinct, D2=%llu symbols (%.1f ms so far)\n", depth, (unsigned long long)N,
                         (unsigned long long)k, maxlen, (unsigned long long)nw, (unsigned long long)ND, tm.ms());
    if (!forced && (ND + k) * 10 > N * 6) { c->arena.release_hi(mk); return PFP_OK; }
    PFP_LAUNCH(c, K_REC_DEDUP, k * 16, k_rs_wid, nblocks(k, BLOCK), (const uint32_t *)eid, (const uint32_t *)slot2id, k, wid, eid , inv0);
    uint32_t *swid, *inv;
    {
        BitRange wr = {0, bits_for(nw ? nw - 1 : 0)};
        PFP_TRY(radix_sort_pairs<uint32_t>(c, wid, inv0, wid1, inv1, k, &wr, 1, &swid, &inv));
        PFP_LAUNCH(c, K_REC_PARSE, k * 4, k_rs_list_bounds, nblocks(k, BLOCK), (const uint32_t *)swid, k, nw, woff);
    }
    const uint32_t *widp = eid;
    uint32_t *D, *wd, *SAD;
    PFP_ALLOC_HI(c, D, uint32_t, ND + 4); PFP_ALLOC_HI(c, wd, uint32_t, ND); PFP_ALLOC_HI(c, SAD, uint32_t, ND);
    PFP_LAUNCH(c, K_REC_PARSE, ND * 12, k_rs_dict_build, nblocks(nw, BLOCK), dS, (const uint32_t *)ps, (const uint32_t *)wrep, (const uint32_t *)wstart, nw, D, wd);
    {
        const size_t mk2 = c->arena.mark_hi();
        uint32_t *rkD; PFP_ALLOC_HI(c, rkD, uint32_t, ND);
        int r2 = 0;
        PFP_TRY(sort_int_suffixes(c, D, ND, maxsym + 2, SAD, rkD, &r2, depth + 1, false));
        c->arena.release_hi(mk2);
    }
    if (verbose) fprintf(stderr, "[pfbwt_hip]   D2 sorted (%.1f ms so far)\n", tm.ms());
    uint32_t *rows, *whole, *rowoff, *wposs, *wrank, *P2, *SA2, *R2, *valid;
    PFP_ALLOC_HI(c, valid, uint32_t, ND); PFP_ALLOC_HI(c, rows, uint32_t, ND); PFP_ALLOC_HI(c, whole, uint32_t, ND); PFP_ALLOC_HI(c, rowoff, uint32_t, ND); PFP_ALLOC_HI(c, wposs, uint32_t, ND);
    PFP_ALLOC_HI(c, wrank, uint32_t, nw); PFP_ALLOC_HI(c, P2, uint32_t, k + 1); PFP_ALLOC_HI(c, SA2, uint32_t, k + 1); PFP_ALLOC_HI(c, R2, uint32_t, k + 1);
    PFP_LAUNCH(c, K_REC_PARSE, ND * 28, k_rs_slots, nblocks(ND, BLOCK), (const uint32_t *)SAD, (const uint32_t *)wd, (const uint32_t *)wstart, (const uint32_t *)woff, ND, rows, whole, valid);
    PFP_TRY((device_scan<uint32_t, 0>(c, whole, wposs, ND, nullptr)));
    PFP_LAUNCH(c, K_REC_PARSE, ND * 16, k_rs_word_ranks, nblocks(ND, BLOCK), (const uint32_t *)SAD, (const uint32_t *)wd, (const uint32_t *)whole, (const uint32_t *)wposs, ND, wrank);
    PFP_LAUNCH(c, K_REC_PARSE, k * 12, k_rs_names, nblocks(k + 1, BLOCK), widp, (const uint32_t *)wrank, k, P2);
    {
        int r2 = 0;
        PFP_TRY(sort_int_suffixes(c, P2, k + 1, nw, SA2, R2, &r2, depth + 1, true));
    }
    if (verbose) fprintf(stderr, "[pfbwt_hip]   P2 sorted (%.1f ms so far)\n", tm.ms());
    uint32_t *ikey = SA2 , *ipos = P2;
    PFP_LAUNCH(c, K_REC_PARSE, k * 20, k_rs_list_payload, nblocks(k, BLOCK), (const uint32_t *)inv, (const uint32_t *)R2, (const uint32_t *)ps, k, ikey, ipos);
    PFP_TRY((device_scan<uint32_t, 0>(c, rows, rowoff, ND, d_cnt + 6)));
    uint32_t R32 = 0; PFP_TRY(d2h_u32(c, d_cnt + 6, &R32));
    if ((uint64_t)R32 != N - 1) { c->arena.release_hi(mk); return PFP_E_CORRUPT; }
    uint32_t *vlist, *head, *chead, *crow;
    PFP_ALLOC_HI(c, vlist, uint32_t, ND); PFP_ALLOC_HI(c, head, uint32_t, ND); PFP_ALLOC_HI(c, chead, uint32_t, ND + 1); PFP_ALLOC_HI(c, crow, uint32_t, ND + 1);
    PFP_TRY(device_compact(c, nullptr, valid, ND, vlist, wposs, d_cnt + 7));
    uint32_t nv32 = 0; PFP_TRY(d2h_u32(c, d_cnt + 7, &nv32));
    const uint64_t nv = nv32;
    uint4 *srec; PFP_ALLOC_HI(c, srec, uint4, nv);
    PFP_LAUNCH(c, K_REC_PARSE, nv * 40, k_rs_heads, nblocks(nv, BLOCK), (const uint32_t *)D, (const uint32_t *)SAD, (const uint32_t *)vlist, nv, head);
    PFP_HIP(c, hipMemsetAsync(d_cnt, 0, 32, c->stream));
    PFP_TRY(device_compact(c, nullptr, head, nv, chead, wposs, d_cnt));
    PFP_LAUNCH(c, K_REC_PARSE, nv * 44, k_rs_slot_records, nblocks(nv, BLOCK), (const uint32_t *)SAD, (const uint32_t *)vlist, (const uint32_t *)rowoff, (const uint32_t *)head, (const uint32_t *)wposs, (const uint32_t *)wd,
               (const uint32_t *)wstart, (const uint32_t *)woff, nv, srec);
    uint32_t nc32 = 0; PFP_TRY(d2h_u32(c, d_cnt, &nc32));
    const uint64_t nc = nc32;
    PFP_LAUNCH(c, K_REC_PARSE, nc * 24, k_rs_class_rows, nblocks(nc + 1, BLOCK), (const uint32_t *)chead, (const uint4 *)srec, nc, nv, N - 1, crow, chead + nc);
    uint32_t tile_rows = c->tun.parse_rec_tile_rows ? c->tun.parse_rec_tile_rows : (uint32_t)RS_TILE;
    if (tile_rows > (uint32_t)RS_TILE) tile_rows = RS_TILE;
    if (tile_rows < 2) tile_rows = 2;
    const int keybits = bits_for(k);
    uint32_t *bigc; PFP_ALLOC_HI(c, bigc, uint32_t, nc + 1);
    const unsigned ga = nblocks(N - 1, RS_TILE / 2);
    if (rank) PFP_LAUNCH(c, K_REC_ASSEMBLE, (N - 1) * 16 + nv * 16, (k_rs_assemble<true, false>), ga, (const uint4 *)srec, (const uint32_t *)chead, (const uint32_t *)crow, (uint32_t)nc, (const uint32_t *)ikey, (const uint32_t *)ipos,
                         keybits, tile_rows, SA, rank, bigc, d_cnt + 1, (uint32_t *)nullptr, (uint8_t *)nullptr);
    else PFP_LAUNCH(c, K_REC_ASSEMBLE, (N - 1) * 12 + nv * 16, (k_rs_assemble<false, false>), ga, (const uint4 *)srec, (const uint32_t *)chead, (const uint32_t *)crow, (uint32_t)nc, (const uint32_t *)ikey, (const uint32_t *)ipos,
                    keybits, tile_rows, SA, rank, bigc, d_cnt + 1, (uint32_t *)nullptr, (uint8_t *)nullptr);
    PFP_LAUNCH(c, K_MISC, 8, k_rs_first_row, 1, SA, rank, N);
    uint32_t nb32 = 0; PFP_TRY(d2h_u32(c, d_cnt + 1, &nb32));
    if (nb32) {
        const uint64_t nb = nb32;
        uint32_t *bigoff; PFP_ALLOC_HI(c, bigoff, uint32_t, nb + 1);
        PFP_LAUNCH(c, K_REC_PARSE, nb * 12, k_rs_big_sizes, nblocks(nb + 1, BLOCK), (const uint32_t *)bigc, nb, (const uint32_t *)crow, bigoff);
        PFP_TRY((device_scan<uint32_t, 0>(c, bigoff, bigoff, nb + 1, d_cnt + 2)));
        uint32_t nbr32 = 0; PFP_TRY(d2h_u32(c, d_cnt + 2, &nbr32));
        const uint64_t nbr = nbr32;
        if (verbose) fprintf(stderr, "[pfbwt_hip]   assembly: %llu classes with more than %u rows (%llu rows) through the global sort\n", (unsigned long long)nb, tile_rows, (unsigned long long)nbr);
        uint64_t *bk0, *bk1; uint32_t *bv0, *bv1;
        PFP_ALLOC_HI(c, bk0, uint64_t, nbr); PFP_ALLOC_HI(c, bk1, uint64_t, nbr); PFP_ALLOC_HI(c, bv0, uint32_t, nbr); PFP_ALLOC_HI(c, bv1, uint32_t, nbr);
        PFP_LAUNCH(c, K_REC_PARSE, nbr * 40, k_rs_big_rows, nblocks(nbr, BLOCK), (const uint32_t *)bigc, (const uint32_t *)bigoff, (uint32_t)nb, nbr, (const uint32_t *)crow, (const uint32_t *)chead, (const uint4 *)srec,
                   (const uint32_t *)ikey, (const uint32_t *)ipos, bk0, bv0, 0);
        BitRange br[2] = {{0, keybits}, {32, 32 + bits_for(nb - 1)}};
        uint64_t *sk; uint32_t *sv;
        PFP_TRY(radix_sort_pairs<uint64_t>(c, bk0, bv0, bk1, bv1, nbr, br, 2, &sk, &sv));
        if (rank) PFP_LAUNCH(c, K_REC_PARSE, nbr * 24, (k_rs_big_store<true, false>), nblocks(nbr, BLOCK), (const uint64_t *)sk, (const uint32_t *)sv, nbr, (const uint32_t *)bigc, (const uint32_t *)bigoff, (const uint32_t *)crow, SA, rank, (uint32_t *)nullptr, (uint8_t *)nullptr);
        else PFP_LAUNCH(c, K_REC_PARSE, nbr * 20, (k_rs_big_store<false, false>), nblocks(nbr, BLOCK), (const uint64_t *)sk, (const uint32_t *)sv, nbr, (const uint32_t *)bigc, (const uint32_t *)bigoff, (const uint32_t *)crow, SA, rank, (uint32_t *)nullptr, (uint8_t *)nullptr);
    }
    PFP_HIP(c, hipStreamSynchronize(c->stream));
    if (verbose) fprintf(stderr, "[pfbwt_hip]   assembled: %llu slots, %llu classes (%.1f ms)\n", (unsigned long long)nv, (unsigned long long)nc, tm.ms());
    c->arena.release_hi(mk);
    *taken = 1;
    return PFP_OK;
}

inline int sort_int_suffixes(pfp_ctx *c, const uint32_t *dS, uint64_t N, uint64_t maxsym, uint32_t *SA, uint32_t *rank, int *rounds, int depth, bool want_rank)
{
    const int mode = c->tun.parse_rec;
    const int max_depth = c->tun.parse_rec_depth > 0 ? c->tun.parse_rec_depth : 1;
    if (mode != 0 && depth < max_depth) {
        const bool shape = N >= c->tun.parse_rec_min && maxsym * 8 <= N;
        if (mode > 0 || shape) {
            int taken = 0;
            PFP_TRY(suffix_sort_pfp(c, dS, N, maxsym, SA, want_rank ? rank : (uint32_t *)nullptr, depth, &taken));
            if (taken) { if (rounds) *rounds = 1; return PFP_OK; }
        }
    }
    return sort_int_suffixes_doubling(c, dS, N, maxsym, SA, rank, rounds);
}

}
```

Baseline: 137.0 Gbases/s.

## Derive occurrence lists from SA(P2) slices and merge-assemble classes instead of LDS sort

In the recursive parse suffix sort, the per-word occurrence lists now come straight from contiguous slices of the sorted P2 suffix array. This drops the radix sort of phrase ids and the inverse list build. Class assembly now uses a merge kernel: each member's pre-sorted slice is placed by binary-searching the other members' key ranges in LDS, replacing the in-LDS radix sort. Batches holding a class with too many members fall back to the old assembly kernel through a list, which adds a host readback and an extra launch.

```diff
diff --git a/pfbwt-f_amd/csrc/common.h b/pfbwt-f_amd/csrc/common.h
--- a/pfbwt-f_amd/csrc/common.h
+++ b/pfbwt-f_amd/csrc/common.h
@@ -116,6 +116,8 @@
     uint64_t parse_rec_min = 1u << 21;
     int parse_rec_depth = 1;
     uint32_t parse_rec_tile_rows = 0;
+    int parse_rec_merge = 1;
+    uint32_t parse_rec_merge_members = 64;
     int dict_rec = -1;
     int dict_rec_p2 = 16;
     int dedup_variant = -1;
diff --git a/pfbwt-f_amd/csrc/dictrec.h b/pfbwt-f_amd/csrc/dictrec.h
--- a/pfbwt-f_amd/csrc/dictrec.h
+++ b/pfbwt-f_amd/csrc/dictrec.h
@@ -372,7 +372,7 @@
     PFP_HIP(c, hipMemsetAsync(cstart, 0, (N + 1) * 4, c->stream));
     const unsigned ga = nblocks(N - 1, RS_TILE / 2);
     PFP_LAUNCH(c, K_REC_ASSEMBLE, (N - 1) * 16 + nv * 16, (k_rs_assemble<false, true>), ga, (const uint4 *)srec, (const uint32_t *)chead, (const uint32_t *)crow, (uint32_t)nc, (const uint32_t *)ikey, (const uint32_t *)ipos,
-               keybits, tile_rows, gsa, (uint32_t *)nullptr, bigc, d_cnt + 1, okey, sflag);
+               keybits, tile_rows, gsa, (uint32_t *)nullptr, bigc, d_cnt + 1, okey, sflag, (const uint32_t *)nullptr);
     PFP_LAUNCH(c, K_MISC, 8, k_rs_first_row, 1, gsa, (uint32_t *)nullptr, N);
     uint32_t nb32 = 0; PFP_TRY(d2h_u32(c, d_cnt + 1, &nb32));
     if (nb32) {
diff --git a/pfbwt-f_amd/csrc/pfbwt_hip.hip b/pfbwt-f_amd/csrc/pfbwt_hip.hip
--- a/pfbwt-f_amd/csrc/pfbwt_hip.hip
+++ b/pfbwt-f_amd/csrc/pfbwt_hip.hip
@@ -89,7 +89,7 @@
 
 static const char *const tunable_names[] = {"verbose", "seg_grid", "seg_stage", "sort_k", "sort_no_table", "class_sort_maxrange", "dedup_table_log2", "no_trigger_table",
                                             "emit_chunk_rows", "fill_subs", "sample_cap", "no_runaware", "big_group_members", "force_wide_rows", "fasta_chunk_bytes", "ingest_block_bytes", "emit_group_rows", "no_slot_records", "dict_text_rounds", "int_key_symbols", "force_run_round",
-                                            "ingest_readers", "expand_dma", "parse_rec", "parse_rec_p2", "parse_rec_min", "parse_rec_depth", "parse_rec_tile_rows", "parse_rec_table_log2", "dict_rec", "dict_rec_p2", "dedup_variant", "dedup_phases", "dedup_period", "dedup_chunk", "doc_lds_max", "dedup_packed", "group_reduce", "scan_waves", "lcp_long_min", "thr_long_min", "thr_tile", "thr_window_rows", "plcp_block_log2", "fill_masks", "fill_skip", "ms_dir_log2", "ms_long_min", "ri_dir_log2", "ri_route"};
+                                            "ingest_readers", "expand_dma", "parse_rec", "parse_rec_p2", "parse_rec_min", "parse_rec_depth", "parse_rec_tile_rows", "parse_rec_merge", "parse_rec_merge_members", "parse_rec_table_log2", "dict_rec", "dict_rec_p2", "dedup_variant", "dedup_phases", "dedup_period", "dedup_chunk", "doc_lds_max", "dedup_packed", "group_reduce", "scan_waves", "lcp_long_min", "thr_long_min", "thr_tile", "thr_window_rows", "plcp_block_log2", "fill_masks", "fill_skip", "ms_dir_log2", "ms_long_min", "ri_dir_log2", "ri_route"};
 static int set_tunable(pfp_ctx *c, const char *key, long long v)
 {
     Tunables &t = c->tun;
@@ -123,6 +123,8 @@
     else if (!strcmp(key, "parse_rec_min")) t.parse_rec_min = v > 0 ? (uint64_t)v : 0;
     else if (!strcmp(key, "parse_rec_depth")) t.parse_rec_depth = (int)v;
     else if (!strcmp(key, "parse_rec_tile_rows")) t.parse_rec_tile_rows = v > 0 ? (uint32_t)v : 0u;
+    else if (!strcmp(key, "parse_rec_merge")) t.parse_rec_merge = v < 0 ? 0 : v > 2 ? 2 : (int)v;
+    else if (!strcmp(key, "parse_rec_merge_members")) t.parse_rec_merge_members = v < 1 ? 1u : v > 1023 ? 1023u : (uint32_t)v;
     else if (!strcmp(key, "parse_rec_table_log2")) t.parse_rec_table_log2 = (int)v;
     else if (!strcmp(key, "dict_rec")) t.dict_rec = (int)v;
     else if (!strcmp(key, "dict_rec_p2")) t.dict_rec_p2 = (int)v;
diff --git a/pfbwt-f_amd/csrc/recsort.h b/pfbwt-f_amd/csrc/recsort.h
--- a/pfbwt-f_amd/csrc/recsort.h
+++ b/pfbwt-f_amd/csrc/recsort.h
@@ -114,6 +114,11 @@
     const uint64_t j = (uint64_t)blockIdx.x * BLOCK + threadIdx.x;
     if (j < k) { const uint32_t id = slot2id[eid[j]]; wid[j] = id; wid_keep[j] = id; idx[j] = (uint32_t)j; }
 }
+__global__ __launch_bounds__(BLOCK) void k_rs_wid_keep(const uint32_t *eid, const uint32_t *slot2id, uint64_t k, uint32_t *wid_keep)
+{
+    const uint64_t j = (uint64_t)blockIdx.x * BLOCK + threadIdx.x;
+    if (j < k) wid_keep[j] = slot2id[eid[j]];
+}
 __global__ __launch_bounds__(BLOCK) void k_rs_dict_build(const uint32_t *S, const uint32_t *ps, const uint32_t *wrep, const uint32_t *wstart, uint64_t nw, uint32_t *D, uint32_t *wd)
 {
     const uint64_t i = (uint64_t)blockIdx.x * BLOCK + threadIdx.x;
@@ -149,6 +154,45 @@
     const uint64_t j = (uint64_t)blockIdx.x * BLOCK + threadIdx.x;
     if (j < k) P2[j] = wrank[wid[j]];
     else if (j == k) P2[j] = 0u;
+}
+__global__ __launch_bounds__(BLOCK) void k_rs_slot_flags(const uint32_t *SAD, const uint32_t *wd, const uint32_t *wstart, uint64_t ND, uint32_t *whole, uint32_t *valid)
+{
+    const uint64_t s = (uint64_t)blockIdx.x * BLOCK + threadIdx.x;
+    if (s >= ND) return;
+    const uint32_t x = SAD[s], i = wd[x], o = x - wstart[i], L = wstart[i + 1] - wstart[i] - 1u;
+    valid[s] = o + 1u < L ? 1u : 0u;
+    whole[s] = o == 0u ? 1u : 0u;
+}
+__global__ __launch_bounds__(BLOCK) void k_rs_slot_rows(const uint32_t *SAD, const uint32_t *wd, const uint32_t *valid, const uint32_t *wrank, const uint32_t *roff, uint64_t ND, uint32_t *rows)
+{
+    const uint64_t s = (uint64_t)blockIdx.x * BLOCK + threadIdx.x;
+    if (s >= ND) return;
+    uint32_t n = 0;
+    if (valid[s]) { const uint32_t r = wrank[wd[SAD[s]]]; n = roff[r + 1] - roff[r]; }
+    rows[s] = n;
+}
+__global__ __launch_bounds__(BLOCK) void k_rs_names_pos(const uint32_t *wid, const uint32_t *wrank, const uint32_t *ps, uint64_t k, uint32_t *P2, uint2 *pp)
+{
+    const uint64_t j = (uint64_t)blockIdx.x * BLOCK + threadIdx.x;
+    if (j < k) { const uint32_t r = wrank[wid[j]]; P2[j] = r; pp[j] = make_uint2(ps[j], r); }
+    else if (j == k) P2[j] = 0u;
+}
+__global__ __launch_bounds__(BLOCK) void k_rs_slice_payload(const uint32_t *SA2, const uint2 *pp, const uint32_t *R2, uint64_t k, uint64_t nw, uint32_t *ikey, uint32_t *ipos, uint32_t *roff)
+{
+    __shared__ uint32_t sr[BLOCK];
+    const uint64_t t = (uint64_t)blockIdx.x * BLOCK + threadIdx.x + 1u;
+    uint32_t r = 0;
+    if (t <= k) {
+        const uint32_t j = SA2[t];
+        const uint2 q = pp[j];
+        r = q.y; ikey[t] = R2[j + 1]; ipos[t] = q.x;
+    }
+    sr[threadIdx.x] = r;
+    __syncthreads();
+    if (t > k) return;
+    const uint32_t rp = threadIdx.x ? sr[threadIdx.x - 1] : (t > 1 ? pp[SA2[t - 1]].y : 0u);
+    if (r != rp) roff[r] = (uint32_t)t;
+    if (t == k) roff[nw + 1] = (uint32_t)(k + 1);
 }
 __global__ __launch_bounds__(BLOCK) void k_rs_list_payload(const uint32_t *inv, const uint32_t *R2, const uint32_t *ps, uint64_t k, uint32_t *ikey, uint32_t *ipos)
 {
@@ -175,12 +219,12 @@
     head[v] = hd;
 }
 __global__ __launch_bounds__(BLOCK) void k_rs_slot_records(const uint32_t *SAD, const uint32_t *vlist, const uint32_t *rowoff, const uint32_t *head, const uint32_t *hpos , const uint32_t *wd, const uint32_t *wstart,
-                                                            const uint32_t *woff, uint64_t nv, uint4 *srec)
+                                                            const uint32_t *woff, const uint32_t *wrank , uint64_t nv, uint4 *srec)
 {
     const uint64_t v = (uint64_t)blockIdx.x * BLOCK + threadIdx.x;
     if (v >= nv) return;
     const uint32_t s = vlist[v], x = SAD[s], i = wd[x];
-    srec[v] = make_uint4(rowoff[s], woff[i], x - wstart[i], hpos[v] + head[v] - 1u);
+    srec[v] = make_uint4(rowoff[s], woff[wrank ? wrank[i] : i], x - wstart[i], hpos[v] + head[v] - 1u);
 }
 __global__ __launch_bounds__(BLOCK) void k_rs_class_rows(const uint32_t *chead, const uint4 *srec, uint64_t nc, uint64_t nv, uint64_t R, uint32_t *crow, uint32_t *chead_end)
 {
@@ -206,10 +250,11 @@
 }
 
 constexpr int RA_DB = 9, RA_RADIX = 1 << RA_DB;
-template <bool RANK, bool KEYOUT> __global__ __launch_bounds__(BLOCK) void k_rs_assemble(const uint4 *srec, const uint32_t *chead , const uint32_t *crow , uint32_t nc,
+template <bool RANK, bool KEYOUT, bool LIST = false> __global__ __launch_bounds__(BLOCK) void k_rs_assemble(const uint4 *srec, const uint32_t *chead , const uint32_t *crow , uint32_t nc,
                                                                             const uint32_t *ikey, const uint32_t *ipos, int keybits, uint32_t tile_rows, uint32_t *SA, uint32_t *rank,
                                                                             uint32_t *bigc, uint32_t *nbig, uint32_t *okey ,
-                                                                            uint8_t *oflag )
+                                                                            uint8_t *oflag ,
+                                                                            const uint32_t *blist )
 {
     constexpr int ITEMS = RS_ITEMS, TILE = RS_TILE;
     constexpr uint32_t STEP = TILE / 2;
@@ -220,11 +265,14 @@
     __shared__ uint32_t red[4];
     __shared__ uint32_t ctl[4];
     const int lane = threadIdx.x & 63, wave = threadIdx.x >> 6;
-    const uint64_t w0 = (uint64_t)blockIdx.x * STEP;
-    if (threadIdx.x == 0) { ctl[0] = rs_lower_bound(crow, 0u, nc, w0); ctl[1] = rs_lower_bound(crow, 0u, nc, w0 + STEP); }
-    __syncthreads();
-    uint32_t ci = ctl[0];
-    const uint32_t ci1 = ctl[1];
+    uint32_t ci, ci1;
+    if (LIST) { ci = blist[2u * blockIdx.x]; ci1 = blist[2u * blockIdx.x + 1u]; }
+    else {
+        const uint64_t w0 = (uint64_t)blockIdx.x * STEP;
+        if (threadIdx.x == 0) { ctl[0] = rs_lower_bound(crow, 0u, nc, w0); ctl[1] = rs_lower_bound(crow, 0u, nc, w0 + STEP); }
+        __syncthreads();
+        ci = ctl[0]; ci1 = ctl[1];
+    }
     while (ci < ci1) {
         __syncthreads();
         if (threadIdx.x == 0) {
@@ -327,6 +375,92 @@
     }
 }
 
+constexpr uint32_t RM_MAX_MEMBERS = 1023;
+template <bool RANK> __global__ __launch_bounds__(BLOCK) void k_rs_merge(const uint4 *srec, const uint32_t *chead , const uint32_t *crow , uint32_t nc, const uint32_t *ikey, const uint32_t *ipos,
+                                                                         uint32_t tile_rows, uint32_t cap, uint32_t *SA, uint32_t *rank, uint32_t *bigc, uint32_t *nbig, uint32_t *fbl, uint32_t *nfb)
+{
+    constexpr int ITEMS = RS_ITEMS, TILE = RS_TILE;
+    constexpr uint32_t STEP = TILE / 2;
+    static_assert(TILE <= 4096, "pk holds 12-bit slot indices");
+    __shared__ uint32_t skey[TILE];
+    __shared__ uint16_t srow[TILE + 1];
+    __shared__ uint32_t ctl[4];
+    const uint64_t w0 = (uint64_t)blockIdx.x * STEP;
+    if (threadIdx.x == 0) { ctl[0] = rs_lower_bound(crow, 0u, nc, w0); ctl[1] = rs_lower_bound(crow, 0u, nc, w0 + STEP); }
+    __syncthreads();
+    uint32_t ci = ctl[0];
+    const uint32_t ci1 = ctl[1];
+    while (ci < ci1) {
+        __syncthreads();
+        if (threadIdx.x == 0) {
+            const uint64_t lim = (uint64_t)crow[ci] + tile_rows;
+            uint32_t lo = ci, hi = ci1;
+            while (lo < hi) { const uint32_t mid = lo + ((hi - lo + 1) >> 1); if ((uint64_t)crow[mid] <= lim) lo = mid; else hi = mid - 1; }
+            ctl[2] = lo; ctl[3] = 0u;
+            if (lo == ci) bigc[atomicAdd(nbig, 1u)] = ci;
+        }
+        __syncthreads();
+        const uint32_t cj = ctl[2];
+        if (cj == ci) { ++ci; continue; }
+        const uint32_t r0 = crow[ci], n = crow[cj] - r0, v0 = chead[ci], ns = chead[cj] - v0;
+        for (uint32_t cc = ci + threadIdx.x; cc < cj; cc += BLOCK) if (chead[cc + 1] - chead[cc] > cap) ctl[3] = 1u;
+        for (uint32_t t = threadIdx.x; t < ns; t += BLOCK) srow[t] = (uint16_t)(srec[v0 + t].x - r0);
+        if (threadIdx.x == 0) srow[ns] = (uint16_t)n;
+        __syncthreads();
+        if (ctl[3]) {
+            if (threadIdx.x == 0) { const uint32_t f = atomicAdd(nfb, 1u); fbl[2u * f] = ci; fbl[2u * f + 1u] = cj; }
+            ci = cj; continue;
+        }
+        uint32_t xi[ITEMS], pk[ITEMS];
+#pragma unroll
+        for (int it = 0; it < ITEMS; ++it) {
+            const uint32_t i = threadIdx.x + (uint32_t)it * BLOCK;
+            xi[it] = 0u; pk[it] = 0u;
+            if (i < n) {
+                uint32_t lo = 0, hi = ns - 1;
+                for (int b = 0; b < 12 && lo < hi; ++b) { const uint32_t mid = lo + ((hi - lo + 1) >> 1); if (srow[mid] <= i) lo = mid; else hi = mid - 1; }
+                const uint4 rec = srec[v0 + lo];
+                const uint32_t e = rec.y + (i - (rec.x - r0));
+                const uint32_t sa = chead[rec.w] - v0, m = chead[rec.w + 1] - chead[rec.w];
+                xi[it] = ipos[e] + rec.z;
+                pk[it] = sa | ((lo - sa) << 12) | (m << 22);
+                if (m > 1u) skey[i] = ikey[e];
+            }
+        }
+        __syncthreads();
+#pragma unroll
+        for (int it = 0; it < ITEMS; ++it) {
+            const uint32_t i = threadIdx.x + (uint32_t)it * BLOCK;
+            if (i < n) {
+                const uint32_t sa = pk[it] & 0xFFFu, me = (pk[it] >> 12) & 0x3FFu, m = pk[it] >> 22;
+                uint32_t place = i;
+                if (m > 1u) {
+                    const uint32_t key = skey[i];
+                    place = (uint32_t)srow[sa] + (i - (uint32_t)srow[sa + me]);
+                    for (uint32_t u = 0; u < m; ++u) {
+                        if (u == me) continue;
+                        const uint32_t a = srow[sa + u];
+                        uint32_t lo = a, hi = srow[sa + u + 1u];
+                        for (int b = 0; b < 12 && lo < hi; ++b) { const uint32_t mid = lo + ((hi - lo) >> 1); if (skey[mid] < key) lo = mid + 1u; else hi = mid; }
+                        place += lo - a;
+                    }
+                }
+                SA[1u + r0 + place] = xi[it];
+                if (RANK) rank[xi[it]] = 1u + r0 + place;
+            }
+        }
+        ci = cj;
+    }
+}
+__global__ __launch_bounds__(BLOCK) void k_rs_member_hist(const uint32_t *chead, const uint32_t *crow, uint64_t nc, unsigned long long *hist)
+{
+    const uint64_t ci = (uint64_t)blockIdx.x * BLOCK + threadIdx.x;
+    if (ci >= nc) return;
+    const uint32_t m = chead[ci + 1] - chead[ci];
+    const int b = m <= 1u ? 0 : m <= 2u ? 1 : m <= 4u ? 2 : m <= 8u ? 3 : m <= 16u ? 4 : m <= 64u ? 5 : 6;
+    atomicAdd(&hist[2 * b], 1ULL); atomicAdd(&hist[2 * b + 1], (unsigned long long)(crow[ci + 1] - crow[ci]));
+}
+
 __global__ __launch_bounds__(BLOCK) void k_rs_big_sizes(const uint32_t *bigc, uint64_t nb, const uint32_t *crow, uint32_t *sizes)
 {
     const uint64_t b = (uint64_t)blockIdx.x * BLOCK + threadIdx.x;
@@ -386,6 +520,7 @@
 {
     *taken = 0;
     const bool forced = c->tun.parse_rec > 0, verbose = c->tun.verbose != 0;
+    const bool slices = c->tun.parse_rec_merge != 0, merge = c->tun.parse_rec_merge == 1;
     const uint32_t p2 = c->tun.parse_rec_p2 >= 2 ? (uint32_t)c->tun.parse_rec_p2 : 4u;
     if (N < 8 || N + 64 >= 0xFFFFFFFFULL || maxsym + 2 >= 0xFFFFFFFFULL) return PFP_OK;
     const size_t mk = c->arena.mark_hi();
@@ -427,9 +562,10 @@
     PFP_TRY(device_compact(c, nullptr, isrep, k, replist, pos, d_cnt + 4));
     uint32_t nw32 = 0; PFP_TRY(d2h_u32(c, d_cnt + 4, &nw32));
     const uint64_t nw = nw32;
-    uint32_t *slot2id, *wrep, *wstart, *wid = isrep , *inv0, *wid1, *inv1, *woff;
+    uint32_t *slot2id, *wrep, *wstart, *wid = isrep , *inv0 = nullptr, *wid1 = nullptr, *inv1 = nullptr, *woff;
     PFP_ALLOC_HI(c, slot2id, uint32_t, tsize); PFP_ALLOC_HI(c, wrep, uint32_t, nw); PFP_ALLOC_HI(c, wstart, uint32_t, nw + 1);
-    PFP_ALLOC_HI(c, inv0, uint32_t, k); PFP_ALLOC_HI(c, wid1, uint32_t, k); PFP_ALLOC_HI(c, inv1, uint32_t, k); PFP_ALLOC_HI(c, woff, uint32_t, nw + 1);
+    if (!slices) { PFP_ALLOC_HI(c, inv0, uint32_t, k); PFP_ALLOC_HI(c, wid1, uint32_t, k); PFP_ALLOC_HI(c, inv1, uint32_t, k); }
+    PFP_ALLOC_HI(c, woff, uint32_t, nw + 2);
     {
         const size_t mk2 = c->arena.mark_hi();
         uint64_t *hk0, *hk1; uint32_t *hv0, *hv1;
@@ -447,9 +583,10 @@
     if (verbose) fprintf(stderr, "[pfbwt_hip] recursive parse sort (depth %d): N=%llu -> %llu phrases (longest %u), %llu distinct, D2=%llu symbols (%.1f ms so far)\n", depth, (unsigned long long)N,
                          (unsigned long long)k, maxlen, (unsigned long long)nw, (unsigned long long)ND, tm.ms());
     if (!forced && (ND + k) * 10 > N * 6) { c->arena.release_hi(mk); return PFP_OK; }
-    PFP_LAUNCH(c, K_REC_DEDUP, k * 16, k_rs_wid, nblocks(k, BLOCK), (const uint32_t *)eid, (const uint32_t *)slot2id, k, wid, eid , inv0);
-    uint32_t *swid, *inv;
-    {
+    if (slices) PFP_LAUNCH(c, K_REC_DEDUP, k * 8, k_rs_wid_keep, nblocks(k, BLOCK), (const uint32_t *)eid, (const uint32_t *)slot2id, k, eid );
+    else PFP_LAUNCH(c, K_REC_DEDUP, k * 16, k_rs_wid, nblocks(k, BLOCK), (const uint32_t *)eid, (const uint32_t *)slot2id, k, wid, eid , inv0);
+    uint32_t *swid, *inv = nullptr;
+    if (!slices) {
         BitRange wr = {0, bits_for(nw ? nw - 1 : 0)};
         PFP_TRY(radix_sort_pairs<uint32_t>(c, wid, inv0, wid1, inv1, k, &wr, 1, &swid, &inv));
         PFP_LAUNCH(c, K_REC_PARSE, k * 4, k_rs_list_bounds, nblocks(k, BLOCK), (const uint32_t *)swid, k, nw, woff);
@@ -466,20 +603,28 @@
         c->arena.release_hi(mk2);
     }
     if (verbose) fprintf(stderr, "[pfbwt_hip]   D2 sorted (%.1f ms so far)\n", tm.ms());
-    uint32_t *rows, *whole, *rowoff, *wposs, *wrank, *P2, *SA2, *R2, *valid;
+    uint32_t *rows, *whole, *rowoff, *wposs, *wrank, *P2, *SA2, *R2, *valid; uint2 *pp = nullptr;
     PFP_ALLOC_HI(c, valid, uint32_t, ND); PFP_ALLOC_HI(c, rows, uint32_t, ND); PFP_ALLOC_HI(c, whole, uint32_t, ND); PFP_ALLOC_HI(c, rowoff, uint32_t, ND); PFP_ALLOC_HI(c, wposs, uint32_t, ND);
     PFP_ALLOC_HI(c, wrank, uint32_t, nw); PFP_ALLOC_HI(c, P2, uint32_t, k + 1); PFP_ALLOC_HI(c, SA2, uint32_t, k + 1); PFP_ALLOC_HI(c, R2, uint32_t, k + 1);
-    PFP_LAUNCH(c, K_REC_PARSE, ND * 28, k_rs_slots, nblocks(ND, BLOCK), (const uint32_t *)SAD, (const uint32_t *)wd, (const uint32_t *)wstart, (const uint32_t *)woff, ND, rows, whole, valid);
+    if (slices) PFP_LAUNCH(c, K_REC_PARSE, ND * 24, k_rs_slot_flags, nblocks(ND, BLOCK), (const uint32_t *)SAD, (const uint32_t *)wd, (const uint32_t *)wstart, ND, whole, valid);
+    else PFP_LAUNCH(c, K_REC_PARSE, ND * 28, k_rs_slots, nblocks(ND, BLOCK), (const uint32_t *)SAD, (const uint32_t *)wd, (const uint32_t *)wstart, (const uint32_t *)woff, ND, rows, whole, valid);
     PFP_TRY((device_scan<uint32_t, 0>(c, whole, wposs, ND, nullptr)));
     PFP_LAUNCH(c, K_REC_PARSE, ND * 16, k_rs_word_ranks, nblocks(ND, BLOCK), (const uint32_t *)SAD, (const uint32_t *)wd, (const uint32_t *)whole, (const uint32_t *)wposs, ND, wrank);
-    PFP_LAUNCH(c, K_REC_PARSE, k * 12, k_rs_names, nblocks(k + 1, BLOCK), widp, (const uint32_t *)wrank, k, P2);
+    if (slices) {
+        PFP_ALLOC_HI(c, pp, uint2, k);
+        PFP_LAUNCH(c, K_REC_PARSE, k * 24, k_rs_names_pos, nblocks(k + 1, BLOCK), widp, (const uint32_t *)wrank, (const uint32_t *)ps, k, P2, pp);
+    } else PFP_LAUNCH(c, K_REC_PARSE, k * 12, k_rs_names, nblocks(k + 1, BLOCK), widp, (const uint32_t *)wrank, k, P2);
     {
         int r2 = 0;
         PFP_TRY(sort_int_suffixes(c, P2, k + 1, nw, SA2, R2, &r2, depth + 1, true));
     }
     if (verbose) fprintf(stderr, "[pfbwt_hip]   P2 sorted (%.1f ms so far)\n", tm.ms());
     uint32_t *ikey = SA2 , *ipos = P2;
-    PFP_LAUNCH(c, K_REC_PARSE, k * 20, k_rs_list_payload, nblocks(k, BLOCK), (const uint32_t *)inv, (const uint32_t *)R2, (const uint32_t *)ps, k, ikey, ipos);
+    if (slices) {
+        PFP_ALLOC_HI(c, ikey, uint32_t, k + 1);
+        PFP_LAUNCH(c, K_REC_PARSE, k * 24, k_rs_slice_payload, nblocks(k, BLOCK), (const uint32_t *)SA2, (const uint2 *)pp, (const uint32_t *)R2, k, nw, ikey, ipos, woff);
+        PFP_LAUNCH(c, K_REC_PARSE, ND * 20, k_rs_slot_rows, nblocks(ND, BLOCK), (const uint32_t *)SAD, (const uint32_t *)wd, (const uint32_t *)valid, (const uint32_t *)wrank, (const uint32_t *)woff, ND, rows);
+    } else PFP_LAUNCH(c, K_REC_PARSE, k * 20, k_rs_list_payload, nblocks(k, BLOCK), (const uint32_t *)inv, (const uint32_t *)R2, (const uint32_t *)ps, k, ikey, ipos);
     PFP_TRY((device_scan<uint32_t, 0>(c, rows, rowoff, ND, d_cnt + 6)));
     uint32_t R32 = 0; PFP_TRY(d2h_u32(c, d_cnt + 6, &R32));
     if ((uint64_t)R32 != N - 1) { c->arena.release_hi(mk); return PFP_E_CORRUPT; }
@@ -493,7 +638,7 @@
     PFP_HIP(c, hipMemsetAsync(d_cnt, 0, 32, c->stream));
     PFP_TRY(device_compact(c, nullptr, head, nv, chead, wposs, d_cnt));
     PFP_LAUNCH(c, K_REC_PARSE, nv * 44, k_rs_slot_records, nblocks(nv, BLOCK), (const uint32_t *)SAD, (const uint32_t *)vlist, (const uint32_t *)rowoff, (const uint32_t *)head, (const uint32_t *)wposs, (const uint32_t *)wd,
-               (const uint32_t *)wstart, (const uint32_t *)woff, nv, srec);
+               (const uint32_t *)wstart, (const uint32_t *)woff, slices ? (const uint32_t *)wrank : (const uint32_t *)nullptr, nv, srec);
     uint32_t nc32 = 0; PFP_TRY(d2h_u32(c, d_cnt, &nc32));
     const uint64_t nc = nc32;
     PFP_LAUNCH(c, K_REC_PARSE, nc * 24, k_rs_class_rows, nblocks(nc + 1, BLOCK), (const uint32_t *)chead, (const uint4 *)srec, nc, nv, N - 1, crow, chead + nc);
@@ -503,10 +648,25 @@
     const int keybits = bits_for(k);
     uint32_t *bigc; PFP_ALLOC_HI(c, bigc, uint32_t, nc + 1);
     const unsigned ga = nblocks(N - 1, RS_TILE / 2);
-    if (rank) PFP_LAUNCH(c, K_REC_ASSEMBLE, (N - 1) * 16 + nv * 16, (k_rs_assemble<true, false>), ga, (const uint4 *)srec, (const uint32_t *)chead, (const uint32_t *)crow, (uint32_t)nc, (const uint32_t *)ikey, (const uint32_t *)ipos,
-                         keybits, tile_rows, SA, rank, bigc, d_cnt + 1, (uint32_t *)nullptr, (uint8_t *)nullptr);
+    uint32_t cap = c->tun.parse_rec_merge_members ? c->tun.parse_rec_merge_members : 1u;
+    if (cap > RM_MAX_MEMBERS) cap = RM_MAX_MEMBERS;
+    uint32_t *fbl = nullptr, *d_nfb = d_cnt + 3;
+    uint32_t nfb = 0;
+    if (merge) {
+        PFP_ALLOC_HI(c, fbl, uint32_t, 2 * (nv / (cap + 1u) + 1u));
+        if (rank) PFP_LAUNCH(c, K_REC_ASSEMBLE, (N - 1) * 16 + nv * 16, (k_rs_merge<true>), ga, (const uint4 *)srec, (const uint32_t *)chead, (const uint32_t *)crow, (uint32_t)nc, (const uint32_t *)ikey, (const uint32_t *)ipos,
+                             tile_rows, cap, SA, rank, bigc, d_cnt + 1, fbl, d_nfb);
+        else PFP_LAUNCH(c, K_REC_ASSEMBLE, (N - 1) * 12 + nv * 16, (k_rs_merge<false>), ga, (const uint4 *)srec, (const uint32_t *)chead, (const uint32_t *)crow, (uint32_t)nc, (const uint32_t *)ikey, (const uint32_t *)ipos,
+                        tile_rows, cap, SA, rank, bigc, d_cnt + 1, fbl, d_nfb);
+        PFP_TRY(d2h_u32(c, d_nfb, &nfb));
+        if (nfb && rank) PFP_LAUNCH(c, K_REC_ASSEMBLE, 0, (k_rs_assemble<true, false, true>), nfb, (const uint4 *)srec, (const uint32_t *)chead, (const uint32_t *)crow, (uint32_t)nc, (const uint32_t *)ikey, (const uint32_t *)ipos,
+                                    keybits, tile_rows, SA, rank, bigc, d_cnt + 1, (uint32_t *)nullptr, (uint8_t *)nullptr, (const uint32_t *)fbl);
+        else if (nfb) PFP_LAUNCH(c, K_REC_ASSEMBLE, 0, (k_rs_assemble<false, false, true>), nfb, (const uint4 *)srec, (const uint32_t *)chead, (const uint32_t *)crow, (uint32_t)nc, (const uint32_t *)ikey, (const uint32_t *)ipos,
+                                 keybits, tile_rows, SA, rank, bigc, d_cnt + 1, (uint32_t *)nullptr, (uint8_t *)nullptr, (const uint32_t *)fbl);
+    } else if (rank) PFP_LAUNCH(c, K_REC_ASSEMBLE, (N - 1) * 16 + nv * 16, (k_rs_assemble<true, false>), ga, (const uint4 *)srec, (const uint32_t *)chead, (const uint32_t *)crow, (uint32_t)nc, (const uint32_t *)ikey, (const uint32_t *)ipos,
+                         keybits, tile_rows, SA, rank, bigc, d_cnt + 1, (uint32_t *)nullptr, (uint8_t *)nullptr, (const uint32_t *)nullptr);
     else PFP_LAUNCH(c, K_REC_ASSEMBLE, (N - 1) * 12 + nv * 16, (k_rs_assemble<false, false>), ga, (const uint4 *)srec, (const uint32_t *)chead, (const uint32_t *)crow, (uint32_t)nc, (const uint32_t *)ikey, (const uint32_t *)ipos,
-                    keybits, tile_rows, SA, rank, bigc, d_cnt + 1, (uint32_t *)nullptr, (uint8_t *)nullptr);
+                    keybits, tile_rows, SA, rank, bigc, d_cnt + 1, (uint32_t *)nullptr, (uint8_t *)nullptr, (const uint32_t *)nullptr);
     PFP_LAUNCH(c, K_MISC, 8, k_rs_first_row, 1, SA, rank, N);
     uint32_t nb32 = 0; PFP_TRY(d2h_u32(c, d_cnt + 1, &nb32));
     if (nb32) {
@@ -528,7 +688,17 @@
         else PFP_LAUNCH(c, K_REC_PARSE, nbr * 20, (k_rs_big_store<false, false>), nblocks(nbr, BLOCK), (const uint64_t *)sk, (const uint32_t *)sv, nbr, (const uint32_t *)bigc, (const uint32_t *)bigoff, (const uint32_t *)crow, SA, rank, (uint32_t *)nullptr, (uint8_t *)nullptr);
     }
     PFP_HIP(c, hipStreamSynchronize(c->stream));
-    if (verbose) fprintf(stderr, "[pfbwt_hip]   assembled: %llu slots, %llu classes (%.1f ms)\n", (unsigned long long)nv, (unsigned long long)nc, tm.ms());
+    if (verbose) {
+        unsigned long long *d_hist, h[14];
+        PFP_ALLOC_HI(c, d_hist, unsigned long long, 14);
+        PFP_HIP(c, hipMemsetAsync(d_hist, 0, sizeof h, c->stream));
+        PFP_LAUNCH(c, K_MISC, nc * 8, k_rs_member_hist, nblocks(nc, BLOCK), (const uint32_t *)chead, (const uint32_t *)crow, nc, d_hist);
+        PFP_HIP(c, hipMemcpyAsync(h, d_hist, sizeof h, hipMemcpyDeviceToHost, c->stream));
+        PFP_HIP(c, hipStreamSynchronize(c->stream));
+        fprintf(stderr, "[pfbwt_hip]   assembled: %llu slots, %llu classes (%.1f ms); lists %s, rows %s; classes / rows by members 1: %llu / %llu, 2: %llu / %llu, 3-4: %llu / %llu, 5-8: %llu / %llu, "
+                        "9-16: %llu / %llu, 17-64: %llu / %llu, >64: %llu / %llu; %u batches with a class of more than %u members sorted\n", (unsigned long long)nv, (unsigned long long)nc, tm.ms(),
+                slices ? "from SA(P2) slices" : "sorted by word", merge ? "merged" : "sorted in LDS", h[0], h[1], h[2], h[3], h[4], h[5], h[6], h[7], h[8], h[9], h[10], h[11], h[12], h[13], nfb, cap);
+    }
     c->arena.release_hi(mk);
     *taken = 1;
     return PFP_OK;
```

Result: faster. 140.3 Gbases/s (median of 6 runs) (+2.4%).
